# Gadersd/whisper-burn

Measured on AMD Instinct MI355X. Metric: real-time factor (audio-sec/wall-sec), higher is better.
Workload: dtype f32; 1 GPU; tiny.en, 30 s of 16 kHz audio per GPU per step, reference windowing (3 windows <= 14.9 s, 3 s overlap), HIP mel + encoder + KV-cached decode, greedy (beam_size 1), max_depth 100; windows=3, beam_size=1, max_depth=100, encoder_gemm_after_the_run=f16x3, parallelism=windows sharded over 1 GPU(s), 1 token all-gather

## Files before the change

### include/whisper_hip.h

```cpp
#ifndef WHISPER_HIP_H
#define WHISPER_HIP_H

#include <stdint.h>

#ifdef __cplusplus
extern "C" {
#endif

typedef enum wb_status {
  WB_OK = 0,
  WB_ERR_ARG = -1,
  WB_ERR_SHAPE = -2,
  WB_ERR_IO = -3,
  WB_ERR_HIP = -4,
  WB_ERR_OOM = -5,
  WB_ERR_STATE = -6
} wb_status;

enum { WB_F32 = 0,
       WB_BF16 = 1 };

typedef struct wb_model wb_model;
typedef struct wb_session wb_session;

// ... 119 lines not shown
                          void* user, int32_t* out_tokens, int32_t row_stride, int32_t* out_lens);

int wb_waveform_to_tokens(wb_model* m, const float* pcm, int64_t n, int sample_rate,
                          const wb_decode_params* p, const uint8_t* is_special, int win_begin,
                          int win_end, int32_t* win_tokens, int32_t row_stride, int32_t* win_lens,
                          int32_t* stitched, int64_t stitched_cap, int64_t* n_stitched);

int wb_waveform_to_tokens_dev(wb_model* m, const float* pcm_dev, int64_t n, int sample_rate,
                              const wb_decode_params* p, const uint8_t* is_special, int win_begin,
                              int win_end, int32_t* win_tokens, int32_t row_stride, int32_t* win_lens,
                              int32_t* stitched, int64_t stitched_cap, int64_t* n_stitched);

typedef int (*wb_allgather_fn)(void* user, const void* send, void* recv, int64_t bytes_per_rank);
typedef struct wb_comm wb_comm;
int wb_comm_unique_id(uint8_t* id128);
int wb_comm_init(const uint8_t* id128, int rank, int world, int device, wb_comm** out);
void wb_comm_free(wb_comm* c);
int wb_comm_allgather(void* comm, const void* send, void* recv, int64_t bytes_per_rank);

int wb_shard_partition(int64_t n_windows, int rank, int world, int64_t* lo, int64_t* hi);

int wb_waveform_to_tokens_sharded(wb_model* m, const float* pcm, int pcm_on_device, int64_t n, int sample_rate,
                                  const wb_decode_params* p, const uint8_t* is_special, int rank, int world,
                                  wb_allgather_fn allgather, void* user, int32_t* win_tokens, int32_t row_stride,
                                  int32_t* win_lens, int64_t win_cap, int32_t* stitched, int64_t stitched_cap,
                                  int64_t* n_stitched);

int64_t wb_window_extents(int64_t n_samples, int sample_rate, int64_t window_len, int overlap_seconds,
                          int64_t* starts, int64_t* lens, int64_t cap);

int wb_find_chunk_overlap(const int32_t* prev, int64_t n_prev, const int32_t* curr, int64_t n_curr,
                          int max_n_offsets, int min_n_overlaps, int64_t* prev_index,
                          int64_t* curr_index);

int wb_stitch_windows(const int32_t* win_tokens, int32_t row_stride, const int32_t* win_lens,
                      int n_windows, int max_n_offsets, int min_n_overlaps, int32_t* out,
                      int64_t cap, int64_t* n_out);

int wb_align_tokens(wb_model* m, const int32_t* tokens, int n, int L, const int32_t* lens, const float* enc, int C,
                    const int32_t* heads, int32_t n_heads, int32_t n_prefix, int32_t drop_last, int32_t filter_width,
                    int32_t* start_pos, float* matrix);
int wb_session_align(wb_session* s, const int32_t* tokens, int32_t row_stride, const int32_t* lens, const int32_t* heads,
                     int32_t n_heads, int32_t n_prefix, int32_t drop_last, int32_t filter_width, int32_t* start_pos,
                     float* matrix);
int wb_dtw_start_positions(int device, const float* x, int32_t N, int32_t C, int32_t* start_pos);
int wb_waveform_to_token_times(wb_model* m, const float* pcm, int64_t n, int sample_rate, const wb_decode_params* p,
                               const uint8_t* is_special, int win_begin, int win_end, int32_t* win_tokens,
                               int32_t row_stride, int32_t* win_lens, int32_t* stitched, int64_t stitched_cap,
                               int64_t* n_stitched, const int32_t* heads, int32_t n_heads, int32_t filter_width,
                               float* win_times, float* stitched_times);
int wb_stitch_windows_times(const int32_t* win_tokens, int32_t row_stride, const int32_t* win_lens, int n_windows,
                            int max_n_offsets, int min_n_overlaps, int32_t* out, int64_t cap, int64_t* n_out,
                            const float* win_times, float* out_times);

int wb_score_tokens(wb_model* m, const int32_t* tokens, int n, int L, const int32_t* lens, const float* enc, int C,
                    const uint8_t* is_special, int32_t mask_until_len, const int32_t* probe_ids, int32_t n_probe,
                    int32_t probe_pos, float* token_logprobs, float* probe_logprobs);
int wb_session_score(wb_session* s, const int32_t* tokens, int32_t row_stride, const int32_t* lens,
                     int32_t mask_until_len, const int32_t* probe_ids, int32_t n_probe, int32_t probe_pos,
                     float* token_logprobs, float* probe_logprobs);
int wb_waveform_detect_language(wb_model* m, const float* pcm, int64_t n, int sample_rate, int32_t padding,
                                int32_t tok_start_of_transcript, const int32_t* lang_ids, int32_t n_lang,
                                int32_t max_windows, float* win_probs, float* mean_probs, int32_t* best);
int wb_waveform_to_token_scores(wb_model* m, const float* pcm, int64_t n, int sample_rate, const wb_decode_params* p,
                                const uint8_t* is_special, int win_begin, int win_end, int32_t* win_tokens,
                                int32_t row_stride, int32_t* win_lens, int32_t* stitched, int64_t stitched_cap,
                                int64_t* n_stitched, int32_t tok_no_speech, float* win_logprobs,
                                float* stitched_logprobs, float* win_avg_logprob, float* win_no_speech_prob);
int wb_logprob_gather(int device, const float* h, int32_t R, int32_t d, const float* E, int32_t V, const float* mask,
                      const uint8_t* row_masked, const int32_t* target, const int32_t* probe_row,
                      const int32_t* probe_id, int32_t n_probe, int32_t v_splits, float* logprob, float* lse,
                      float* probe_lp);

typedef struct wb_sample_params {
  float temperature;
  int32_t best_of;
  uint64_t seed;
  int32_t attempt;
} wb_sample_params;
void wb_sample_params_default(wb_sample_params* p);
int wb_session_rewind(wb_session* s);
int wb_session_graph_count(const wb_session* s);
int64_t wb_session_graph_captures(const wb_session* s);
int wb_session_decode_sample(wb_session* s, const wb_decode_params* p, const wb_sample_params* sp, const int32_t* prompt,
                             int32_t prompt_len, const uint8_t* active, const int32_t* stream_ids, int32_t* out_tokens,
                             int32_t row_stride, int32_t* out_lens, double* out_sum_logprob, int32_t* out_best);

int wb_session_last_samples(wb_session* s, int32_t* tokens, int32_t row_stride, int32_t* lens);

enum { WB_FALLBACK_MAX_TEMPERATURES = 8 };
enum { WB_FALLBACK_ACCEPT = 0, WB_FALLBACK_RETRY = 1, WB_FALLBACK_NO_SPEECH = 2 };
typedef struct wb_fallback_params {
  float temperatures[WB_FALLBACK_MAX_TEMPERATURES];
  int32_t n_temperatures;
  int32_t best_of;
  float logprob_threshold;
  float no_speech_threshold;
  float compression_ratio_threshold;
  uint64_t seed;
  int32_t tok_no_speech;
} wb_fallback_params;
void wb_fallback_params_default(wb_fallback_params* p);
int wb_fallback_decide(const wb_fallback_params* fp, float avg_logprob, float no_speech_prob, float ratio);
typedef double (*wb_ratio_fn)(void* user, const int32_t* tokens, int32_t n);
int wb_waveform_to_tokens_fallback(wb_model* m, const float* pcm, int64_t n, int sample_rate, const wb_decode_params* p,
                                   const uint8_t* is_special, int win_begin, int win_end, int32_t* win_tokens,
                                   int32_t row_stride, int32_t* win_lens, int32_t* stitched, int64_t stitched_cap,
                                   int64_t* n_stitched, const wb_fallback_params* fp, wb_ratio_fn ratio, void* user,
                                   float* win_temperature, int32_t* win_status, float* win_avg_logprob,
                                   float* win_no_speech_prob, float* win_ratio, int32_t* win_attempts);
int wb_sample_rows(int device, const float* logits, int32_t R, int32_t ld, int32_t V, const float* mask,
                   const uint8_t* row_masked, const float* row_stats, float temperature, uint64_t seed, int32_t attempt,
                   const int32_t* stream, const int32_t* position, int32_t eot, int32_t* out_token, float* out_logprob,
                   int32_t* out_err);

int64_t wb_first_repetition_end(const int32_t* tokens, int64_t n, int64_t period);
int64_t wb_repetition_period(const int32_t* tokens, int64_t n, int64_t min_repetitions);
int wb_find_repeated_tokens_index(const int32_t* tokens, int64_t n, int64_t window_size, int64_t min_repeat_count,
                                  int64_t* first_repeat_index, int64_t* end);

int wb_mel_constants(double sample_rate, float* hann400, float* filters_80x201);

int wb_mel_dft_table(float* table_402x400);


int wb_profile_enable(int on);
int wb_profile_read(double* out8, int reset);

typedef struct wb_kernel_stat {
  char name[96];
  int64_t calls;
  double total_ms;
  double algo_bytes;
} wb_kernel_stat;
int wb_profile_kernels(wb_kernel_stat* out, int cap, int reset);

const char* wb_last_error(void);
const char* wb_version(void);

#ifdef __cplusplus
}
#endif
#endif
```

### rust/whisper-hip/src/ffi.rs

```rust
#![allow(non_camel_case_types)]
use std::os::raw::{c_char, c_double, c_float, c_int, c_void};

#[repr(C)]
pub struct wb_model {
    _private: [u8; 0],
}
#[repr(C)]
pub struct wb_session {
    _private: [u8; 0],
}
#[repr(C)]
pub struct wb_comm {
    _private: [u8; 0],
}

#[repr(C)]
#[derive(Default, Clone, Copy, Debug, PartialEq, Eq)]
pub struct wb_dims {
    pub n_mels: i32,
    pub n_audio_ctx: i32,
    pub n_audio_state: i32,
    pub n_audio_head: i32,
    pub n_audio_layer: i32,
    pub n_vocab: i32,
// ... 43 lines not shown
    pub tok_no_speech: i32,
}

pub type wb_ratio_fn = Option<unsafe extern "C" fn(user: *mut c_void, tokens: *const i32, n: i32) -> c_double>;

pub const WB_OK: c_int = 0;
pub const WB_ERR_ARG: c_int = -1;
pub const WB_ERR_SHAPE: c_int = -2;
pub const WB_ERR_IO: c_int = -3;
pub const WB_ERR_HIP: c_int = -4;
pub const WB_ERR_OOM: c_int = -5;
pub const WB_ERR_STATE: c_int = -6;
pub const WB_F32: c_int = 0;
pub const WB_BF16: c_int = 1;
pub const WB_FRONTEND_FFT: c_int = 0;
pub const WB_FRONTEND_REFERENCE: c_int = 1;

extern "C" {
    pub fn wb_model_load_dump_dir(dir: *const c_char, device: c_int, compute_dtype: c_int, out: *mut *mut wb_model) -> c_int;
    pub fn wb_model_load_burn_record(mpk_gz_path: *const c_char, cfg_path: *const c_char, device: c_int,
                                     compute_dtype: c_int, out: *mut *mut wb_model) -> c_int;
    pub fn wb_model_dims(m: *const wb_model, out: *mut wb_dims) -> c_int;
    pub fn wb_model_free(m: *mut wb_model);
    pub fn wb_model_set_frame_limit(m: *mut wb_model, whisper_geometry: c_int) -> c_int;
    pub fn wb_model_set_frontend(m: *mut wb_model, frontend: c_int) -> c_int;
    pub fn wb_model_frontend(m: *const wb_model) -> c_int;
    pub fn wb_model_encoder_gemm(m: *const wb_model) -> c_int;
    pub fn wb_model_decoder_gemm(m: *const wb_model) -> c_int;
    pub fn wb_max_waveform_samples(n_frame_max: i64) -> i64;
    pub fn wb_prep_audio(device: c_int, pcm: *const c_float, n: i64, sample_rate: c_double, mel: *mut c_float,
                         n_frames: *mut i64) -> c_int;
    pub fn wb_prep_audio_frontend(device: c_int, pcm: *const c_float, n: i64, sample_rate: c_double, mel: *mut c_float,
                                  n_frames: *mut i64, frontend: c_int) -> c_int;
    pub fn wb_mel_dft_table(table_402x400: *mut c_float) -> c_int;
    pub fn wb_forward_encoder(m: *mut wb_model, mel: *const c_float, b: c_int, t: c_int, out: *mut c_float) -> c_int;
    pub fn wb_forward_decoder(m: *mut wb_model, tokens: *const i32, n: c_int, l: c_int, enc: *const c_float, c: c_int,
                              logits: *mut c_float) -> c_int;
    pub fn wb_forward(m: *mut wb_model, mel: *const c_float, b: c_int, t: c_int, tokens: *const i32, l: c_int,
                      logits: *mut c_float) -> c_int;
    pub fn wb_decode_params_default(p: *mut wb_decode_params);
    pub fn wb_window_extents(n_samples: i64, sample_rate: c_int, window_len: i64, overlap_seconds: c_int,
                             starts: *mut i64, lens: *mut i64, cap: i64) -> i64;
    pub fn wb_waveform_to_tokens(m: *mut wb_model, pcm: *const c_float, n: i64, sample_rate: c_int,
                                 p: *const wb_decode_params, is_special: *const u8, win_begin: c_int, win_end: c_int,
                                 win_tokens: *mut i32, row_stride: i32, win_lens: *mut i32, stitched: *mut i32,
                                 stitched_cap: i64, n_stitched: *mut i64) -> c_int;
    pub fn wb_align_tokens(m: *mut wb_model, tokens: *const i32, n: c_int, L: c_int, lens: *const i32, enc: *const c_float,
                           C: c_int, heads: *const i32, n_heads: i32, n_prefix: i32, drop_last: i32, filter_width: i32,
                           start_pos: *mut i32, matrix: *mut c_float) -> c_int;
    pub fn wb_session_align(s: *mut wb_session, tokens: *const i32, row_stride: i32, lens: *const i32, heads: *const i32,
                            n_heads: i32, n_prefix: i32, drop_last: i32, filter_width: i32, start_pos: *mut i32,
                            matrix: *mut c_float) -> c_int;
    pub fn wb_dtw_start_positions(device: c_int, x: *const c_float, N: i32, C: i32, start_pos: *mut i32) -> c_int;
    pub fn wb_waveform_to_token_times(m: *mut wb_model, pcm: *const c_float, n: i64, sample_rate: c_int,
                                      p: *const wb_decode_params, is_special: *const u8, win_begin: c_int, win_end: c_int,
                                      win_tokens: *mut i32, row_stride: i32, win_lens: *mut i32, stitched: *mut i32,
                                      stitched_cap: i64, n_stitched: *mut i64, heads: *const i32, n_heads: i32,
                                      filter_width: i32, win_times: *mut c_float, stitched_times: *mut c_float) -> c_int;
    pub fn wb_stitch_windows_times(win_tokens: *const i32, row_stride: i32, win_lens: *const i32, n_windows: c_int,
                                   max_n_offsets: c_int, min_n_overlaps: c_int, out: *mut i32, cap: i64, n_out: *mut i64,
                                   win_times: *const c_float, out_times: *mut c_float) -> c_int;
    pub fn wb_score_tokens(m: *mut wb_model, tokens: *const i32, n: c_int, L: c_int, lens: *const i32, enc: *const c_float,
                           C: c_int, is_special: *const u8, mask_until_len: i32, probe_ids: *const i32, n_probe: i32,
                           probe_pos: i32, token_logprobs: *mut c_float, probe_logprobs: *mut c_float) -> c_int;
    pub fn wb_session_score(s: *mut wb_session, tokens: *const i32, row_stride: i32, lens: *const i32, mask_until_len: i32,
                            probe_ids: *const i32, n_probe: i32, probe_pos: i32, token_logprobs: *mut c_float,
                            probe_logprobs: *mut c_float) -> c_int;
    pub fn wb_waveform_detect_language(m: *mut wb_model, pcm: *const c_float, n: i64, sample_rate: c_int, padding: i32,
                                       tok_start_of_transcript: i32, lang_ids: *const i32, n_lang: i32, max_windows: i32,
                                       win_probs: *mut c_float, mean_probs: *mut c_float, best: *mut i32) -> c_int;
    pub fn wb_waveform_to_token_scores(m: *mut wb_model, pcm: *const c_float, n: i64, sample_rate: c_int,
                                       p: *const wb_decode_params, is_special: *const u8, win_begin: c_int, win_end: c_int,
                                       win_tokens: *mut i32, row_stride: i32, win_lens: *mut i32, stitched: *mut i32,
                                       stitched_cap: i64, n_stitched: *mut i64, tok_no_speech: i32,
                                       win_logprobs: *mut c_float, stitched_logprobs: *mut c_float,
                                       win_avg_logprob: *mut c_float, win_no_speech_prob: *mut c_float) -> c_int;
    pub fn wb_logprob_gather(device: c_int, h: *const c_float, R: i32, d: i32, E: *const c_float, V: i32,
                             mask: *const c_float, row_masked: *const u8, target: *const i32, probe_row: *const i32,
                             probe_id: *const i32, n_probe: i32, v_splits: i32, logprob: *mut c_float, lse: *mut c_float,
                             probe_lp: *mut c_float) -> c_int;
    pub fn wb_session_rewind(s: *mut wb_session) -> c_int;
    pub fn wb_session_graph_count(s: *const wb_session) -> c_int;
    pub fn wb_session_graph_captures(s: *const wb_session) -> i64;
    pub fn wb_session_last_samples(s: *mut wb_session, tokens: *mut i32, row_stride: i32, lens: *mut i32) -> c_int;
    pub fn wb_sample_rows(device: c_int, logits: *const c_float, R: i32, ld: i32, V: i32, mask: *const c_float,
                          row_masked: *const u8, row_stats: *const c_float, temperature: c_float, seed: u64, attempt: i32,
                          stream: *const i32, position: *const i32, eot: i32, out_token: *mut i32,
                          out_logprob: *mut c_float, out_err: *mut i32) -> c_int;
    pub fn wb_session_begin(m: *mut wb_model, pcm: *const c_float, n_pcm: i64, starts: *const i64, lens: *const i64,
                            n_windows: c_int, max_beams: c_int, padding: c_int, out: *mut *mut wb_session) -> c_int;
    pub fn wb_session_set_special_mask(s: *mut wb_session, is_special: *const u8) -> c_int;
    pub fn wb_session_step(s: *mut wb_session, new_tokens: *const i32, parent: *const i32, window: *const i32, n: c_int,
                           apply_special_mask: c_int, k: c_int, top_ids: *mut i32, top_logprobs: *mut c_float) -> c_int;
    pub fn wb_session_decode(s: *mut wb_session, p: *const wb_decode_params, out_tokens: *mut i32, row_stride: i32,
                             out_lens: *mut i32) -> c_int;
    pub fn wb_session_free(s: *mut wb_session);
    pub fn wb_wav_read_f32(path: *const c_char, out: *mut c_float, capacity: i64, n_samples: *mut i64) -> c_int;
    pub fn wb_wav_read_f32_any_rate(path: *const c_char, out: *mut c_float, capacity: i64, n_samples: *mut i64) -> c_int;
    pub fn wb_resample_len(n_in: i64, rate_in: i32, rate_out: i32) -> i64;
    pub fn wb_resample_dev(device: c_int, src_dev: *const c_float, n_in: i64, rate_in: i32, rate_out: i32,
                           dst_dev: *mut c_float, capacity: i64, n_out: *mut i64) -> c_int;
    pub fn wb_comm_unique_id(id128: *mut u8) -> c_int;
    pub fn wb_comm_init(id128: *const u8, rank: c_int, world: c_int, device: c_int, out: *mut *mut wb_comm) -> c_int;
    pub fn wb_comm_free(c: *mut wb_comm);
    pub fn wb_comm_allgather(comm: *mut c_void, send: *const c_void, recv: *mut c_void, bytes_per_rank: i64) -> c_int;
    pub fn wb_shard_partition(n_windows: i64, rank: c_int, world: c_int, lo: *mut i64, hi: *mut i64) -> c_int;
    pub fn wb_waveform_to_tokens_sharded(m: *mut wb_model, pcm: *const c_float, pcm_on_device: c_int, n: i64,
                                         sample_rate: c_int, p: *const wb_decode_params, is_special: *const u8,
                                         rank: c_int, world: c_int, allgather: wb_allgather_fn, user: *mut c_void,
                                         win_tokens: *mut i32, row_stride: i32, win_lens: *mut i32, win_cap: i64,
                                         stitched: *mut i32, stitched_cap: i64, n_stitched: *mut i64) -> c_int;
    pub fn wb_last_error() -> *const c_char;
    pub fn wb_version() -> *const c_char;
}

extern "C" {
    pub fn wb_sample_params_default(p: *mut wb_sample_params);
    pub fn wb_session_decode_sample(s: *mut wb_session, p: *const wb_decode_params, sp: *const wb_sample_params,
                                    prompt: *const i32, prompt_len: i32, active: *const u8, stream_ids: *const i32,
                                    out_tokens: *mut i32, row_stride: i32, out_lens: *mut i32,
                                    out_sum_logprob: *mut c_double, out_best: *mut i32) -> c_int;
    pub fn wb_fallback_params_default(p: *mut wb_fallback_params);
    pub fn wb_fallback_decide(fp: *const wb_fallback_params, avg_logprob: c_float, no_speech_prob: c_float,
                              ratio: c_float) -> c_int;
    pub fn wb_waveform_to_tokens_fallback(m: *mut wb_model, pcm: *const c_float, n: i64, sample_rate: c_int,
                                          p: *const wb_decode_params, is_special: *const u8, win_begin: c_int,
                                          win_end: c_int, win_tokens: *mut i32, row_stride: i32, win_lens: *mut i32,
                                          stitched: *mut i32, stitched_cap: i64, n_stitched: *mut i64,
                                          fp: *const wb_fallback_params, ratio: wb_ratio_fn, user: *mut c_void,
                                          win_temperature: *mut c_float, win_status: *mut i32,
                                          win_avg_logprob: *mut c_float, win_no_speech_prob: *mut c_float,
                                          win_ratio: *mut c_float, win_attempts: *mut i32) -> c_int;
}

pub type wb_allgather_fn = Option<unsafe extern "C" fn(user: *mut c_void, send: *const c_void, recv: *mut c_void,
                                                       bytes_per_rank: i64) -> c_int>;

pub unsafe extern "C" fn wb_comm_allgather_thunk(user: *mut c_void, send: *const c_void, recv: *mut c_void,
                                                  bytes_per_rank: i64) -> c_int {
    wb_comm_allgather(user, send, recv, bytes_per_rank)
}

pub type wb_user = *mut c_void;
```

### whisper-burn_amd/csrc/decode.h

```cpp
#pragma once
#include <hip/hip_runtime.h>
#include <hip/hip_ext.h>
#include <stdint.h>

#include <algorithm>

#include "kernels.h"
#include "wb_internal.h"

namespace wb {

constexpr int MAX_BEAMS = 8;
constexpr int TOPK_MAX = 8;
constexpr int CA_STRIDE = 66;
constexpr int CA_NCH_MAX = 12;
constexpr int TS_STRIDE = 2 + 2 * TOPK_MAX;
constexpr int GV_CT = 128;
constexpr int GV_CT_LOGITS = 128;
constexpr int KS_MAX = 16;

enum { ST_N = 0, ST_STEP = 1, ST_HDR = 4 };
enum { GC_STEP = 0, GC_NDONE = 1, GC_ALLDONE = 2, GC_BAD = 3, GC_HDR = 4 };
struct StepLayout {
  int S = 0, W = 0;
// ... 153 lines not shown
};
void launch_sample_rows(hipStream_t st, const SampleRowsArgs& a);

struct MlpFusedArgs {
  const int* st = nullptr; int S = 0, d = 0;
  const float* x_in = nullptr; const float* pend = nullptr; int KSp = 0; const float* pbias = nullptr; float* x_out = nullptr;
  int n_head = 0, n_chunks = 0;
  const float* ln_g = nullptr; const float* ln_b = nullptr; float ln_eps = 0.f; int ln_inside = 0;
  const float* W1 = nullptr; int ld1 = 0; const float* b1 = nullptr;
  const float* W2 = nullptr;
  float* P = nullptr;
  unsigned long long* stamps = nullptr;
  int row0 = 0;
  const void* g_x_in = nullptr; const void* g_pend = nullptr; void* g_x_out = nullptr; void* g_P = nullptr;
};
struct AttnFusedArgs {
  const int* st = nullptr; StepLayout lay; int S = 0, d = 0, n_head = 0;
  const float* x_in = nullptr; const float* pend = nullptr; int KSp = 0; const float* pbias = nullptr; float* x_out = nullptr;
  const float* ln_g = nullptr; const float* ln_b = nullptr; float ln_eps = 0.f; int ln_inside = 0;
  const float* Wqkv = nullptr; int ldqkv = 0; const float* bqkv = nullptr; float scale = 0.f;
  float* Kc = nullptr; float* Vc = nullptr; const int* tabs = nullptr; int Lmax = 0;
  const float* Wo = nullptr;
  float* P = nullptr;
  unsigned long long* stamps = nullptr;
  const void* g_x_in = nullptr; const void* g_pend = nullptr; void* g_x_out = nullptr; void* g_P = nullptr;
};
struct CrossFusedArgs {
  const int* st = nullptr; StepLayout lay; int S = 0, d = 0, n_head = 0;
  const float* x_in = nullptr; const float* pend = nullptr; int KSp = 0; const float* pbias = nullptr; float* x_out = nullptr;
  const float* ln_g = nullptr; const float* ln_b = nullptr; float ln_eps = 0.f; int ln_inside = 0;
  const float* Wq = nullptr; const float* bq = nullptr; float scale = 0.f;
  const float* ckv = nullptr; int ldkv = 0, koff = 0;
  const int* win_row0 = nullptr; const int* win_C = nullptr;
  int n_pass = 1;
  const float* Wo = nullptr;
  float* P = nullptr;
  unsigned long long* stamps = nullptr;
  const void* g_x_in = nullptr; const void* g_pend = nullptr; void* g_x_out = nullptr; void* g_P = nullptr;
};
struct SkinnyArgs {
  const float* A = nullptr; int lda = 0;
  const float* B = nullptr; int ldb = 0;
  int M = 0, N = 0, K = 0, ksplit = 1;
  float* P = nullptr; int plane = 0;
  const uint16_t* Bh = nullptr; const uint16_t* Bl = nullptr;
  int* range_flag = nullptr;
  const int* st = nullptr;
};
void launch_split_weight_f16_tiles(hipStream_t st, const float* W, int K, int N, uint16_t* hi, uint16_t* lo);
int skinny_ksplit(int K, int N, int max_ks, int max_rows);
bool skinny_supported(int M, int K, int N);
int launch_dec_skinny_gemm(hipStream_t st, const SkinnyArgs& a);

struct PsLayerArgs { AttnFusedArgs attn; CrossFusedArgs cross; MlpFusedArgs mlp; };
enum { PSR_ATTN = 0, PSR_CROSS = 1, PSR_MLP = 2, PSR_LOGITS = 3, PSR_MERGE = 4, PSR_FINLN = 5 };
struct PsRole { int kind, layer, a, b; };
constexpr int PS_MAX_FORCED = 8;
struct PersistArgs {
  const PsLayerArgs* layers = nullptr;
  const PsRole* roles = nullptr; int n_roles = 0;
  const int* role_off = nullptr;
  const int* res_role = nullptr;
  int n_logits_roles = 0;
  int n_layer = 0, n_rows = 0, S = 0, d = 0, n_head = 0, nb_mlp = 0;
  int n_pass = 1;
  int* ctl = nullptr;
  int step0 = 0, n_steps = 0;
  int n_forced = 0; int forced[PS_MAX_FORCED] = {0, 0, 0, 0, 0, 0, 0, 0};
  int mask_until_len = 0;
  const void* x_fin = nullptr; const void* P2 = nullptr; const float* b2_last = nullptr;
  void* g_xn = nullptr;
  unsigned tag_base = 0;
  const float* ln_g = nullptr; const float* ln_b = nullptr; float ln_eps = 0.f; int ln_inside = 0;
  const float* Et = nullptr; int vocab_ld = 0, V = 0; const float* mask = nullptr;
  float* tstats = nullptr; int n_tiles = 0;
  int* gctl = nullptr; int* gtok = nullptr; int Lmax = 0, eot = 0;
  const float* E = nullptr; const float* pos = nullptr; void* x0 = nullptr; int* tabs = nullptr;
  int* dead = nullptr;
  unsigned long long* stamps = nullptr;
};
int ps_ctl_ints(int S, int n_layer);
bool dec_persist_supported(int d, int n_rows, int max_keys);
int dec_persist_resident_slots(int d, int n_rows, int max_keys);
int dec_persist_max_grid(int device, int d, int n_rows, int max_keys);
int launch_dec_persist(hipStream_t st, const PersistArgs& a, int grid);
void launch_ps_seed(hipStream_t st, const float* x, int n, void* gx, unsigned tag);

#if defined(HIPEMU) && !defined(HIPEMU_PROD_GEOMETRY)
constexpr int CROSS_FUSED_MAX_C = 384;
#else
constexpr int CROSS_FUSED_MAX_C = 768;
#endif
constexpr int CROSS_FUSED_MAX_PASSES = 2;
void launch_dec_cross_fused(hipStream_t st, const CrossFusedArgs& a, int n_rows_hint);
bool dec_fused_supported(int d);
int dec_mlp_fused_planes(int d);
void launch_dec_mlp_fused(hipStream_t st, const MlpFusedArgs& a, int n_rows_hint);
void launch_dec_attn_fused(hipStream_t st, const AttnFusedArgs& a, int n_rows_hint);

}
```

### whisper-burn_amd/csrc/decode_chain.cpp

```cpp
#include <climits>
#include <cstring>

#include "decode_step.h"
#include "handoff.h"
#include "switches.h"

using namespace wb;

namespace wb {

static int run_persistent_chain(wb_session* s, int eot, int max_depth, int mask_until_len, const int32_t* forced, int n_forced,
                                int* steps_done, bool* fell_back) {
  *fell_back = false;
  WB_REQUIRE(n_forced >= 0 && n_forced <= PS_MAX_FORCED, WB_ERR_ARG, "persistent decode: %d prompt steps", n_forced);
  const char* inject = sw::persist_inject_fail();
  wb_model* m = s->m;
  const wb_dims& D = m->dims;
  const int d = D.n_text_state, H = D.n_text_head, NL = D.n_text_layer, V = D.n_vocab, S = s->S, W = s->W;
  const StepLayout& L = s->lay;
  hipStream_t st = s->st;
  const int NB = dec_mlp_fused_planes(d);
  const int n_tiles = (V + 127) / 128;
  const size_t pool = (size_t)s->Lmax * S;
  const int ldkv = 2 * d;
  WB_REQUIRE(NB <= 32 && H <= 8, WB_ERR_SHAPE, "persistent decode: more planes than its folds hold");
  WB_TRY(s->ps_gx.ensure_zeroed(((size_t)2 * S + 8) * d * 8, st));
  WB_TRY(s->ps_gpa.ensure_zeroed(((size_t)H * S + 8) * d * 8, st));
  WB_TRY(s->ps_gpc.ensure_zeroed(((size_t)H * S + 8) * d * 8, st));
  WB_TRY(s->ps_gp2.ensure_zeroed(((size_t)NB * S + 8) * d * 8, st));
  WB_TRY(s->ps_gxn.ensure_zeroed(((size_t)S + 8) * d * 8, st));
  if (((s->ps_launches + 1) & 0xffffu) == 0) {
    for (DevMem* b : {&s->ps_gx, &s->ps_gpa, &s->ps_gpc, &s->ps_gp2, &s->ps_gxn}) WB_HIP(hipMemsetAsync(b->p, 0, b->bytes, st));
    s->ps_launches++;
  }
  const unsigned tag_base = ((++s->ps_launches) & 0xffffu) << 16;
  char* gxb[2] = {static_cast<char*>(s->ps_gx.p), static_cast<char*>(s->ps_gx.p) + (size_t)S * d * 8};
  std::vector<PsLayerArgs> la(NL);
  float* xb[2] = {s->x.as<float>(), s->x.as<float>() + (size_t)S * d};
  int xi = 0;
  for (int l = 0; l < NL; l++) {
    const DecBlockW& b = m->dec[l];
    AttnFusedArgs& fa = la[l].attn;
    fa.st = s->state.as<int>(); fa.lay = L; fa.S = S; fa.d = d; fa.n_head = H;
    fa.x_in = xb[xi]; fa.pend = l == 0 ? nullptr : s->P2.as<float>(); fa.KSp = l == 0 ? 0 : NB;
    fa.pbias = l == 0 ? nullptr : m->dec[l - 1].mlp2.b; fa.x_out = xb[xi ^ 1];
    fa.ln_g = b.ln1.g; fa.ln_b = b.ln1.b; fa.ln_eps = b.ln1.eps; fa.ln_inside = m->ln_eps_inside_sqrt;
    fa.Wqkv = b.qkv.w; fa.ldqkv = b.qkv.n; fa.bqkv = b.qkv.b; fa.scale = m->qk_scale;
    fa.Kc = s->kc.as<float>() + (size_t)l * pool * d; fa.Vc = s->vc.as<float>() + (size_t)l * pool * d;
    fa.tabs = s->tabs.as<int>(); fa.Lmax = s->Lmax; fa.Wo = b.out.w; fa.P = s->Pa.as<float>();
    fa.g_x_in = gxb[xi]; fa.g_pend = l == 0 ? nullptr : s->ps_gp2.p; fa.g_x_out = gxb[xi ^ 1]; fa.g_P = s->ps_gpa.p;
    xi ^= 1;
    CrossFusedArgs& ca = la[l].cross;
    ca.st = s->state.as<int>(); ca.lay = L; ca.S = S; ca.d = d; ca.n_head = H;
    ca.x_in = xb[xi]; ca.pend = s->Pa.as<float>(); ca.KSp = H; ca.pbias = b.out.b; ca.x_out = xb[xi ^ 1];
    ca.ln_g = b.ln2.g; ca.ln_b = b.ln2.b; ca.ln_eps = b.ln2.eps; ca.ln_inside = m->ln_eps_inside_sqrt;
    ca.Wq = b.cq.w; ca.bq = b.cq.b; ca.scale = m->qk_scale;
    ca.ckv = s->ckv.as<float>() + (size_t)l * s->enc_rows * 2 * d; ca.ldkv = ldkv; ca.koff = 0;
    ca.win_row0 = s->win_meta.as<int>(); ca.win_C = s->win_meta.as<int>() + W;
    ca.Wo = b.cout.w; ca.P = s->Pc.as<float>();
    ca.n_pass = s->maxC > CROSS_FUSED_MAX_C ? 2 : 1;
    ca.g_x_in = gxb[xi]; ca.g_pend = s->ps_gpa.p; ca.g_x_out = gxb[xi ^ 1]; ca.g_P = s->ps_gpc.p;
    xi ^= 1;
    MlpFusedArgs& ma = la[l].mlp;
    ma.st = s->state.as<int>(); ma.S = S; ma.d = d;
    ma.x_in = xb[xi]; ma.pend = s->Pc.as<float>(); ma.KSp = H; ma.pbias = b.cout.b; ma.x_out = xb[xi ^ 1];
    ma.ln_g = b.ln3.g; ma.ln_b = b.ln3.b; ma.ln_eps = b.ln3.eps; ma.ln_inside = m->ln_eps_inside_sqrt;
    ma.W1 = b.mlp1.w; ma.ld1 = b.mlp1.n; ma.b1 = b.mlp1.b; ma.W2 = b.mlp2.w; ma.P = s->P2.as<float>();
    ma.g_x_in = gxb[xi]; ma.g_pend = s->ps_gpc.p; ma.g_x_out = gxb[xi ^ 1]; ma.g_P = s->ps_gp2.p;
    xi ^= 1;
  }
  std::vector<PsRole> lr;
  for (int l = 0; l < NL; l++) {
    for (int r = 0; r < W; r++) for (int h = 0; h < H; h++) lr.push_back(PsRole{PSR_ATTN, l, h, r});
    for (int r = 0; r < W; r++) for (int h = 0; h < H; h++) lr.push_back(PsRole{PSR_CROSS, l, h, r});
    for (int j = 0; j < NB; j++) lr.push_back(PsRole{PSR_MLP, l, j, 0});
  }
  const int grid = std::max(1, std::min(s->ps_grid, (int)lr.size() + n_tiles + 2 * W));
  std::vector<std::vector<PsRole>> deal(grid);
  for (size_t i = 0; i < lr.size(); i++) deal[i % grid].push_back(lr[i]);
  std::vector<int> cand;
  for (int b = 0; b < grid; b++) {
    bool early = false;
    for (const PsRole& r : deal[b]) early |= r.layer == 0 && (r.kind == PSR_ATTN || r.kind == PSR_CROSS);
    if (!early) cand.push_back(b);
  }
  if ((int)cand.size() * 4 < n_tiles) { cand.clear(); for (int b = 0; b < grid; b++) cand.push_back(b); }
  std::vector<char> is_fin(grid, 0);
  {
    std::vector<int> order(grid);
    for (int b = 0; b < grid; b++) order[b] = b;
    std::stable_sort(order.begin(), order.end(), [&](int x, int y) { return deal[x].size() < deal[y].size(); });
    for (int r = 0; r < W; r++) { deal[order[r % grid]].push_back(PsRole{PSR_FINLN, 0, 0, r}); is_fin[order[r % grid]] = 1; }
  }
  if ((int)cand.size() > 2 * W) cand.erase(std::remove_if(cand.begin(), cand.end(), [&](int b) { return is_fin[b] != 0; }), cand.end());
  std::stable_sort(cand.begin(), cand.end(), [&](int x, int y) { return deal[x].size() < deal[y].size(); });
  const int tpb = (n_tiles + (int)cand.size() - 1) / (int)cand.size();
  const int n_lg = (n_tiles + tpb - 1) / tpb;
  for (int q = 0; q < n_lg; q++)
    deal[cand[q]].push_back(PsRole{PSR_LOGITS, q, q * tpb, std::min(tpb, n_tiles - q * tpb)});
  {
    std::vector<int> order(grid);
    for (int b = 0; b < grid; b++) order[b] = b;
    std::stable_sort(order.begin(), order.end(), [&](int x, int y) { return deal[x].size() < deal[y].size(); });
    for (int r = 0; r < W; r++) deal[order[r % grid]].push_back(PsRole{PSR_MERGE, 0, 0, r});
  }
  std::vector<PsRole> roles;
  std::vector<int> role_off(grid + 1, 0);
  for (int b = 0; b < grid; b++) {
    role_off[b] = (int)roles.size();
    roles.insert(roles.end(), deal[b].begin(), deal[b].end());
  }
  role_off[grid] = (int)roles.size();
  const char* res_sw = sw::persist_resident();
  const bool res_on = !(res_sw && res_sw[0] == '0') && dec_persist_resident_slots(d, W, s->maxC) > 0;
  std::vector<int> res_role(grid, -1);
  int n_res = 0;
  if (res_on)
    for (int b = 0; b < grid; b++) {
      int n_layer_roles = 0, at = -1;
      for (int i = role_off[b]; i < role_off[b + 1]; i++)
        if (roles[i].kind <= PSR_MLP) { n_layer_roles++; at = i; }
      if (n_layer_roles == 1 && roles[at].kind != PSR_MLP) { res_role[b] = at; n_res++; }
    }
  if (res_sw && !strcmp(res_sw, "log")) fprintf(stderr, "persist resident blocks: %d of %d\n", n_res, grid);
  const int n_ctl = ps_ctl_ints(S, NL);
  WB_TRY(s->ps_layers.ensure(la.size() * sizeof(PsLayerArgs)));
  WB_TRY(s->ps_roles.ensure(roles.size() * sizeof(PsRole) + (role_off.size() + res_role.size()) * 4));
  WB_TRY(s->ps_ctl.ensure((size_t)n_ctl * 4));
  WB_TRY(s->ps_dead.ensure((size_t)S * 4));
  WB_TRY(s->ps_tstats.ensure((size_t)S * n_tiles * 2 * 4));
  std::vector<int> ctl0(n_ctl, 0);
  ctl0[HX_STOP] = INT_MAX;
  WB_HIP(hipMemcpyAsync(s->ps_layers.p, la.data(), la.size() * sizeof(PsLayerArgs), hipMemcpyHostToDevice, st));
  WB_HIP(hipMemcpyAsync(s->ps_roles.p, roles.data(), roles.size() * sizeof(PsRole), hipMemcpyHostToDevice, st));
  WB_HIP(hipMemcpyAsync(static_cast<char*>(s->ps_roles.p) + roles.size() * sizeof(PsRole) + role_off.size() * 4, res_role.data(),
                        res_role.size() * 4, hipMemcpyHostToDevice, st));
  WB_HIP(hipMemcpyAsync(static_cast<char*>(s->ps_roles.p) + roles.size() * sizeof(PsRole), role_off.data(), role_off.size() * 4,
                        hipMemcpyHostToDevice, st));
  WB_HIP(hipMemcpyAsync(s->ps_ctl.p, ctl0.data(), (size_t)n_ctl * 4, hipMemcpyHostToDevice, st));
  WB_HIP(hipMemsetAsync(s->ps_dead.p, 0, (size_t)S * 4, st));
  PersistArgs a;
  a.layers = s->ps_layers.as<PsLayerArgs>(); a.roles = s->ps_roles.as<PsRole>(); a.n_roles = (int)roles.size();
  a.role_off = reinterpret_cast<const int*>(static_cast<char*>(s->ps_roles.p) + roles.size() * sizeof(PsRole));
  if (n_res > 0) a.res_role = a.role_off + role_off.size();
  a.n_logits_roles = n_lg;
  a.n_layer = NL; a.n_rows = W; a.S = S; a.d = d; a.n_head = H; a.nb_mlp = NB;
  a.n_pass = s->maxC > CROSS_FUSED_MAX_C ? 2 : 1;
  a.ctl = s->ps_ctl.as<int>(); a.step0 = s->step; a.n_steps = n_forced + max_depth; a.mask_until_len = mask_until_len;
  a.n_forced = n_forced;
  for (int i = 0; i < n_forced; i++) a.forced[i] = forced[i];
  a.g_xn = s->ps_gxn.p;
  a.x_fin = gxb[xi]; a.P2 = s->ps_gp2.p; a.b2_last = m->dec[NL - 1].mlp2.b; a.tag_base = tag_base;
  a.ln_g = m->ln_dec.g; a.ln_b = m->ln_dec.b; a.ln_eps = m->ln_dec.eps; a.ln_inside = m->ln_eps_inside_sqrt;
  a.Et = m->tok_emb_t; a.vocab_ld = m->vocab_ld; a.V = V; a.mask = s->mask.as<float>();
  a.tstats = s->ps_tstats.as<float>(); a.n_tiles = n_tiles;
  a.gctl = s->gctl.as<int>(); a.gtok = s->gtok.as<int>(); a.Lmax = s->Lmax; a.eot = eot;
  a.E = m->tok_emb; a.pos = m->dec_pos; a.x0 = gxb[0]; a.tabs = s->tabs.as<int>(); a.dead = s->ps_dead.as<int>();
  const char* stamps_path = sw::ps_stamps();
  const size_t n_stamps = stamps_path ? (size_t)(n_forced + max_depth) * roles.size() * 8 : 0;
  if (n_stamps) {
    WB_TRY(s->ps_stamps.ensure(n_stamps * 8));
    WB_HIP(hipMemsetAsync(s->ps_stamps.p, 0, n_stamps * 8, st));
    a.stamps = s->ps_stamps.as<unsigned long long>();
  }
  WB_REQUIRE(3 * NL * (n_forced + max_depth + 1) + 4 < 0x10000, WB_ERR_SHAPE,
             "persistent decode: %d layers x %d steps do not fit the 16-bit granule tags", NL, max_depth);
  launch_dec_prepare(st, reinterpret_cast<const int*>(s->host_block_dev), s->state.as<int>(), L, W, s->tabs.as<int>(),
                     s->Lmax, m->tok_emb, m->dec_pos, d, s->x.as<float>(), s->gctl.as<int>());
  launch_ps_seed(st, s->x.as<float>(), W * d, gxb[0], tag_base + 1u);
  WB_HIP(hipStreamSynchronize(st));
  hipEvent_t e0 = nullptr, e1 = nullptr;
  prof_tag(KC_PERSIST, 0.0);
  const bool timed = prof_take_events(&e0, &e1);
  if (timed) WB_HIP(hipEventRecord(e0, st));
  const bool refused = (inject && !strcmp(inject, "launch")) || launch_dec_persist(st, a, grid) != 0;
  if (timed) WB_HIP(hipEventRecord(e1, st));
  if (refused) {
    (void)hipGetLastError();
    s->ps_grid = 0;
    *fell_back = true;
    *steps_done = 0;
    return WB_OK;
  }
  std::vector<int> ctl(n_ctl);
  WB_HIP(hipMemcpyAsync(ctl.data(), s->ps_ctl.p, (size_t)n_ctl * 4, hipMemcpyDeviceToHost, st));
  int gstep = 0;
  WB_HIP(hipMemcpyAsync(&gstep, s->gctl.as<int>() + GC_STEP, 4, hipMemcpyDeviceToHost, st));
  WB_HIP(hipStreamSynchronize(st));
  if (ctl[HX_ERR] != 0 && gstep == s->step) {
    s->ps_grid = 0;
    *fell_back = true;
    *steps_done = 0;
    return WB_OK;
  }
  WB_REQUIRE(ctl[HX_ERR] == 0, WB_ERR_HIP, "persistent decode: a wait gave up (counter %d) at step %d", ctl[HX_ERR] - 1, gstep);
  if (n_stamps) {
    std::vector<unsigned long long> hs(n_stamps);
    WB_HIP(hipMemcpy(hs.data(), s->ps_stamps.p, n_stamps * 8, hipMemcpyDeviceToHost));
    if (FILE* f = fopen(stamps_path, "wb")) {
      const int hdr[4] = {n_forced + max_depth, (int)roles.size(), grid, 8};
      fwrite(hdr, 4, 4, f);
      std::vector<int> kinds(roles.size());
      for (size_t i = 0; i < roles.size(); i++)
        kinds[i] = roles[i].kind | ((roles[i].kind <= PSR_MLP ? roles[i].layer : 0) << 8) |
                   ((roles[i].kind == PSR_LOGITS ? 0 : roles[i].b) << 16);
      fwrite(kinds.data(), 4, kinds.size(), f);
      fwrite(hs.data(), 8, hs.size(), f);
      fclose(f);
    }
  }
  *steps_done = std::max(0, std::min(n_forced + max_depth, gstep - s->step));
  return WB_OK;
}

int session_greedy_chain(wb_session* s, const int32_t* prompt, int eot, int max_depth, int mask_until_len, int prompt_len,
                         int32_t* out_tokens, int32_t row_stride, int32_t* out_lens) {
  wb_model* m = s->m;
  const int S = s->S, W = s->W;
  WB_REQUIRE(S == W, WB_ERR_STATE, "chained greedy decode needs max_beams == 1");
  WB_REQUIRE(prompt && prompt_len >= 1, WB_ERR_ARG, "chained greedy decode: empty prompt");
  WB_REQUIRE(s->step == 0 || (s->prev_n == W && s->step == prompt_len - 1), WB_ERR_STATE,
             "chained greedy decode: the session is neither fresh nor prefilled");
  const int n_forced_max = prompt_len - 1;
  auto host_prefill = [&]() -> int {
    std::vector<int32_t> tok(W), par(W), win(W);
    for (int t = s->step; t < prompt_len - 1; t++) {
      for (int w = 0; w < W; w++) { tok[w] = prompt[t]; par[w] = t == 0 ? -1 : w; win[w] = w; }
      WB_TRY(wb_session_step(s, tok.data(), par.data(), win.data(), W, 0, 0, nullptr, nullptr));
    }
    return WB_OK;
  };
  WB_REQUIRE(s->has_mask || mask_until_len < prompt_len || max_depth == 0, WB_ERR_STATE,
             "wb_session_decode: special mask not set");
  const int asked_depth = max_depth;
  max_depth = std::min(max_depth, s->Lmax - (prompt_len - 1));
  WB_HIP(hipSetDevice(m->device));
  hipStream_t st = s->st;
  const size_t ctl_ints = GC_HDR + 3 * (size_t)S;
  WB_TRY(s->gctl.ensure(ctl_ints * 4));
  WB_TRY(s->gtok.ensure(((size_t)S * s->Lmax + 1) * 4));
  std::vector<int> ctl(ctl_ints, 0);
  auto seed_ctl = [&]() -> int {
    std::fill(ctl.begin(), ctl.end(), 0);
    ctl[GC_STEP] = s->step;
    for (int i = 0; i < W; i++) ctl[GC_HDR + i] = prompt[s->step];
    WB_HIP(hipMemcpyAsync(s->gctl.p, ctl.data(), ctl_ints * 4, hipMemcpyHostToDevice, st));
    WB_HIP(hipStreamSynchronize(st));
    return WB_OK;
  };
  const StepPlan plan = plan_step(s, W, false);
  const int n_launch = plan.n_launch;
  const bool fuse_ln = plan.fuse_ln;
  const int chunk = 16;
  int depth = 0;
  bool persist = plan.persist && max_depth > 0;
  if (persist) {
    if (s->ps_grid < 0) s->ps_grid = dec_persist_max_grid(m->device, m->dims.n_text_state, W, s->maxC);
    persist = s->ps_grid > 0;
  }
  int n_forced = 0;
  if (persist && sw::persist_prefill() && s->step == 0 && n_forced_max <= PS_MAX_FORCED && s->has_mask) n_forced = n_forced_max;
  if (n_forced == 0) WB_TRY(host_prefill());
  WB_TRY(seed_ctl());
  ScopedTimer tm(st, 3);
  if (persist) {
    bool fell_back = false;
    WB_TRY(run_persistent_chain(s, eot, max_depth, mask_until_len, prompt + s->step + 1, n_forced, &depth, &fell_back));
    if (fell_back) {
      persist = false;
      depth = 0;
      WB_TRY(host_prefill());
      WB_TRY(seed_ctl());
      n_forced = 0;
    } else {
      if (profile().on) profile().ms[4] += depth;
      depth -= n_forced;
      s->step += n_forced;
      s->prev_n = W;
      s->prev_win.resize(W);
      for (int w = 0; w < W; w++) s->prev_win[w] = w;
    }
  }
  if (!persist) {
  if (fuse_ln)
    launch_dec_prepare(st, reinterpret_cast<const int*>(s->host_block_dev), s->state.as<int>(), s->lay, n_launch,
                       s->tabs.as<int>(), s->Lmax, m->tok_emb, m->dec_pos, m->dims.n_text_state, s->x.as<float>(),
                       s->gctl.as<int>());
  const bool speculate = fuse_ln && sw::speculate();
  if (speculate && !s->st2) {
    WB_HIP(hipStreamCreateWithFlags(&s->st2, hipStreamNonBlocking));
    WB_HIP(hipEventCreateWithFlags(&s->ev_seg, hipEventDisableTiming));
  }
  auto enqueue_segment = [&](int* enq) -> int {
    int n = 0;
    while (depth + n < max_depth && n < chunk) {
      const int d0 = depth + n;
      const int use_mask = (prompt_len + d0) <= mask_until_len ? 1 : 0;
      const int run = (!use_mask && max_depth - d0 >= chunk) ? chunk : 1;
      StepCall call;
      call.k = 1; call.use_mask = use_mask; call.chained = true; call.eot = eot; call.reps = run;
      WB_TRY(launch_step(s, plan, call));
      if (profile().on) profile().ms[4] += run;
      n += run;
    }
    *enq = n;
    return WB_OK;
  };
  auto read_flags = [&](bool behind_event) -> int {
    if (behind_event) {
      WB_HIP(hipStreamWaitEvent(s->st2, s->ev_seg, 0));
      WB_HIP(hipMemcpyAsync(ctl.data(), s->gctl.p, ctl_ints * 4, hipMemcpyDeviceToHost, s->st2));
      WB_HIP(hipStreamSynchronize(s->st2));
    } else {
      WB_HIP(hipMemcpyAsync(ctl.data(), s->gctl.p, ctl_ints * 4, hipMemcpyDeviceToHost, st));
      WB_HIP(hipStreamSynchronize(st));
    }
    return WB_OK;
  };
  auto all_done = [&]() {
    bool d = true;
    for (int i = 0; i < W; i++) d = d && ctl[GC_HDR + S + i] != 0;
    return d;
  };
  const bool poll = fuse_ln && sw::poll() && !profile().on;
  volatile int* hfl = reinterpret_cast<volatile int*>(s->host_block + s->chain_flags_off);
  if (poll) for (int i = 0; i < 2 * S; i++) hfl[i] = 0;
  auto wait_flags = [&](int want_step, bool* done) -> int {
    for (long spins = 0;; spins++) {
      bool ready = true;
      for (int i = 0; i < W && ready; i++) ready = hfl[2 * i] >= want_step;
      if (ready) break;
      bool fin = true;
      for (int i = 0; i < W && fin; i++) fin = hfl[2 * i + 1] != 0;
      if (fin) break;
      if ((spins & 0xfff) == 0xfff) {
        const hipError_t q = hipStreamQuery(st);
        if (q == hipSuccess) {
          bool r2 = true;
          for (int i = 0; i < W && r2; i++) r2 = hfl[2 * i] >= want_step;
          if (r2) break;
          bool all = true;
          for (int i = 0; i < W; i++) all = all && hfl[2 * i + 1] != 0;
          if (all) break;
          set_error("chained decode: the device stopped at step %d of %d", (int)hfl[0], want_step);
          return WB_ERR_HIP;
        }
        if (q != hipErrorNotReady) { set_error("chained decode: %s", hipGetErrorString(q)); return WB_ERR_HIP; }
      }
    }
    __atomic_thread_fence(__ATOMIC_ACQUIRE);
    bool all = true;
    for (int i = 0; i < W; i++) all = all && hfl[2 * i + 1] != 0;
    *done = all;
    return WB_OK;
  };
  if (!speculate) {
    while (depth < max_depth) {
      int n = 0;
      WB_TRY(enqueue_segment(&n));
      depth += n;
      if (poll) {
        bool done = false;
        WB_TRY(wait_flags(s->step + depth, &done));
        if (done) break;
      } else {
        WB_TRY(read_flags(false));
        if (all_done()) break;
      }
    }
  } else {
    int n_cur = 0;
    WB_TRY(enqueue_segment(&n_cur));
    depth += n_cur;
    while (true) {
      WB_HIP(hipEventRecord(s->ev_seg, st));
      int n_next = 0;
      if (depth < max_depth) { WB_TRY(enqueue_segment(&n_next)); depth += n_next; }
      WB_TRY(read_flags(true));
      if (all_done() || n_next == 0) break;
    }
    WB_HIP(hipStreamSynchronize(st));
  }
  }
  tm.stop();
  std::vector<int> toks((size_t)S * s->Lmax + 1);
  WB_HIP(hipMemcpyAsync(ctl.data(), s->gctl.p, ctl_ints * 4, hipMemcpyDeviceToHost, st));
  WB_HIP(hipMemcpyAsync(toks.data(), s->gtok.p, toks.size() * 4, hipMemcpyDeviceToHost, st));
  WB_HIP(hipStreamSynchronize(st));
  tm.collect();
  WB_TRY(dec_split_check(s));
  WB_REQUIRE(ctl[GC_BAD] == 0, WB_ERR_STATE, "a decode step produced a row without a finite log-prob (NaN logits: non-finite "
             "weights or activations); its window was ended on <|endoftext|> on the device and the rows of this call are invalid");
  for (int w = 0; w < W; w++) {
    int len = ctl[GC_HDR + 2 * S + w];
    if (len < prompt_len) len = prompt_len;
    len = std::min(len, prompt_len + max_depth);
    WB_REQUIRE(len <= row_stride, WB_ERR_ARG, "row_stride too small");
    for (int p = prompt_len; p < len; p++) out_tokens[(size_t)w * row_stride + p] = toks[(size_t)w * s->Lmax + p];
    out_lens[w] = len;
  }
  if (profile().on && !persist && s->prof_cls_cross >= 0 && s->prof_cls_self >= 0) {
    const int dm = m->dims.n_text_state, NL = m->dims.n_text_layer;
    double dead_ckv = 0, dead_self = 0;
    for (int w = 0; w < W; w++) {
      const int live = std::max(0, std::min(out_lens[w] - prompt_len, depth));
      for (int t = live; t < depth; t++) { dead_ckv += 8.0 * s->C[w] * dm; dead_self += 8.0 * (s->step + t + 1) * dm; }
    }
    prof_adjust_bytes(s->prof_cls_cross, -(double)NL * dead_ckv);
    prof_adjust_bytes(s->prof_cls_self, -(double)NL * dead_self);
  }
  if (profile().on && persist) {
    const double dm = m->dims.n_text_state, NL = m->dims.n_text_layer;
    double bytes = (double)(depth + n_forced) * 4.0 * NL * 14.0 * dm * dm + (double)depth * 4.0 * (double)m->dims.n_vocab * dm;
    for (int w = 0; w < W; w++)
      for (int t = 0; t < n_forced; t++) bytes += NL * (8.0 * s->C[w] * dm + 8.0 * (t + 1) * dm);
    for (int w = 0; w < W; w++) {
      const int live = std::max(0, std::min(out_lens[w] - prompt_len, depth));
      for (int t = 0; t < live; t++) bytes += NL * (8.0 * s->C[w] * dm + 8.0 * (s->step + t + 1) * dm);
    }
    prof_adjust_bytes(KC_PERSIST, bytes);
  }
  s->prof_step_off = 0;
  s->step += depth;
  s->prev_len.assign(W, s->step);
  s->last_had_logits = 0;
  if (max_depth < asked_depth)
    for (int w = 0; w < W; w++)
      WB_REQUIRE(ctl[GC_HDR + S + w] != 0, WB_ERR_SHAPE, "Token sequence length %d must not exceed %d.", s->Lmax + 1,
                 s->Lmax);
  return WB_OK;
}
}
```

### whisper-burn_amd/csrc/decode_fused_bodies.h

```cpp
#pragma once
#include <hip/hip_runtime.h>

#include "decode.h"
#include "handoff.h"
#include "wave_ops.h"

namespace wb {
namespace fused {

struct PsStep {
  const unsigned* ctr = nullptr; unsigned target = 0; int ctr_index = 0;
  const int* ctl = nullptr;
  int step = 0;
  int n_rows = 0;
  const int* dead = nullptr;
  int* lds_flag = nullptr;
  unsigned long long* stamp = nullptr;
  int n_ctr = 1;
  unsigned tag_in = 0, tag_out = 0;
  bool known_dead = false;
  mutable bool saw_dead = false;
};
constexpr int PS_STAMPS = 8;
__device__ __forceinline__ void ps_stamp(const PsStep& ps, int k) {
// ... 12 lines not shown
                               : hx_wait(ps.ctr, ps.target, ps.ctl, ps.step, ps.ctr_index, ps.lds_flag);
  ps_stamp(ps, 1);
  return ok;
}
__device__ __forceinline__ bool ps_sweep_retry(unsigned& sweeps, const PsStep& ps) {
  if ((sweeps & 31u) == 31u &&
      (__hip_atomic_load(ps.ctl + HX_STOP, __ATOMIC_RELAXED, __HIP_MEMORY_SCOPE_AGENT) <= ps.step ||
       __hip_atomic_load(ps.ctl + HX_ERR, __ATOMIC_RELAXED, __HIP_MEMORY_SCOPE_AGENT) != 0)) return true;
  if (++sweeps > HX_SWEEP_LIMIT) {
    __hip_atomic_store(const_cast<int*>(ps.ctl) + HX_ERR, 5000 + ps.ctr_index, __ATOMIC_RELAXED, __HIP_MEMORY_SCOPE_AGENT);
    return true;
  }
  __builtin_amdgcn_s_sleep(1);
  return false;
}
__device__ __forceinline__ bool ps_sweeps_ok(const PsStep& ps) { return *ps.lds_flag != 0; }
template <int UNITS>
__device__ __forceinline__ void ps_nap() {
#if !defined(WB_PS_DRY) || defined(WB_PS_DRY_NAPS)
#ifndef WB_PS_NAP_ADJ
#define WB_PS_NAP_ADJ 0
#endif
#pragma unroll
  for (int i = 0; i < UNITS + (WB_PS_NAP_ADJ); i++) __builtin_amdgcn_s_sleep(64);
#endif
}

#ifdef WB_STAMPS
#define WB_STAMP_DECL unsigned long long stamp_buf[16];
#define WB_STAMP(i) do { if (threadIdx.x == 0 && blockIdx.x == 0 && blockIdx.y == 0) sm.stamp_buf[i] = wall_clock64(); } while (0)
#define WB_STAMP_FLUSH(a, n) do { if (threadIdx.x == 0 && blockIdx.x == 0 && blockIdx.y == 0 && (a).stamps) for (int _i = 0; _i < (n); _i++) (a).stamps[_i] = sm.stamp_buf[_i]; } while (0)
#else
#define WB_STAMP_DECL
#define WB_STAMP(i) do {} while (0)
#define WB_STAMP_FLUSH(a, n) do {} while (0)
#endif

constexpr int FD_MAX = 512;
constexpr int FA_MAXPOS = 448;


constexpr int ROLE_NT = 512;
template <int MR, int DPL, bool REC>
struct MlpLds {
  static constexpr int d = 64 * DPL, HS = 64, G = d / 4 <= 32 ? 8 : 4;
  alignas(16) float hs[MR][d];
  alignas(16) float red[8][MR][HS];
  alignas(16) float hid[MR][HS];
  alignas(16) float obuf[(G - 1) * MR * d];
  float mlb[REC ? MR : 1][48][2];
  float coef[REC ? MR : 1][48];
  WB_STAMP_DECL
};
template <int DPL>
struct AttnLds {
  static constexpr int d = 64 * DPL, G = d / 4 <= 32 ? 8 : 4;
  static constexpr int RED = (8 * 192 > (G - 1) * d) ? 8 * 192 : (G - 1) * d;
  alignas(16) float hs[d];
  alignas(16) float red[RED];
  alignas(16) float qkv[192];
  int tbs[FA_MAXPOS];
  float sc[FA_MAXPOS];
  alignas(16) float part[32][64];
  alignas(16) float att[64];
  WB_STAMP_DECL
};
template <int DPL, int NP>
struct CrossLds {
  static constexpr int d = 64 * DPL, G = d / 4 <= 32 ? 8 : 4, CMAX = NP * CROSS_FUSED_MAX_C;
  alignas(16) float hs[d];
  alignas(16) float red[8][64];
  alignas(16) float qv[64];
  float sc[CMAX];
  float pbuf[CMAX];
  alignas(16) float part[32][64];
  alignas(16) float att[64];
  alignas(16) float obuf[(G - 1) * d];
};

template <int DPL, int NP, int RS>
struct ResGeom {
  static constexpr int d = 64 * DPL, G = d / 4 <= 32 ? 8 : 4, RPG = 64 / G;
  static constexpr int KW = d / 8, RK = DPL >= 6 ? 8 : 16, NIT = KW / RK;
  static constexpr int NRND = (NIT - 2 < RS / RK ? NIT - 2 : RS / RK) > 0 ? (NIT - 2 < RS / RK ? NIT - 2 : RS / RK) : 0;
  static constexpr int WO_A = NRND * RK;
  static constexpr int NWO_A = RS - WO_A < RPG ? RS - WO_A : RPG;
  static constexpr int SL = 4, NTILE = CROSS_FUSED_MAX_C / 128;
  static constexpr int NVT = NP > 1 ? 0 : (RS / SL < NTILE ? RS / SL : NTILE);
  static constexpr int WO_X = NVT * SL;
  static constexpr int NWO_X = NP > 1 ? 0 : (RS - WO_X < RPG ? RS - WO_X : RPG);
  static_assert(RS >= 0 && WO_A + NWO_A <= RS && WO_X + NWO_X <= RS, "resident slots");
};
__device__ __forceinline__ float4 res_ld(const float4* res, int slot, int tid) { return res[slot * ROLE_NT + tid]; }
__device__ __forceinline__ void res_st(float4* res, int slot, int tid, const float4& v) { res[slot * ROLE_NT + tid] = v; }

__device__ __forceinline__ float gelu_erf_f(float x) {
  return 0.5f * x * (1.0f + erff(x * 0.70710678118654752440f));
}

template <int DPL>
__device__ __forceinline__ void fold_ln_row(const float* __restrict__ x_in, const float* __restrict__ pend, int KSp,
                                            int64_t plane, const float* __restrict__ pbias, float* __restrict__ x_out,
                                            const float* __restrict__ g, const float* __restrict__ b, float eps,
                                            int eps_inside, int d, int row, int lane, float* __restrict__ out) {
  int co[DPL];
#pragma unroll
  for (int i = 0; i < DPL; i++) co[i] = lane + (64 * i < d ? 64 * i : 0);
  float gv[DPL], bv[DPL], v[DPL];
  const float* xr = x_in + (int64_t)row * d;
#pragma unroll
  for (int i = 0; i < DPL; i++) { gv[i] = g[co[i]]; bv[i] = b[co[i]]; v[i] = xr[co[i]]; }
  if (KSp > 0) {
    float acc[DPL];
#pragma unroll
    for (int i = 0; i < DPL; i++) acc[i] = pbias[co[i]];
    const float* pp = pend + (int64_t)row * d;
    constexpr int CH = DPL <= 6 ? 8 : 4;
    for (int sp = 0; sp < KSp; sp += CH) {
      float t[CH][DPL];
#pragma unroll
      for (int j = 0; j < CH; j++) {
        const float* pj = pp + (int64_t)min(sp + j, KSp - 1) * plane;
#pragma unroll
        for (int i = 0; i < DPL; i++) t[j][i] = pj[co[i]];
      }
#pragma unroll
      for (int j = 0; j < CH; j++) {
        const bool live = sp + j < KSp;
#pragma unroll
        for (int i = 0; i < DPL; i++) acc[i] += live ? t[j][i] : 0.f;
      }
    }
#pragma unroll
    for (int i = 0; i < DPL; i++) v[i] = v[i] + acc[i];
  }
  float s = 0.f;
#pragma unroll
  for (int i = 0; i < DPL; i++) {
    if (64 * i < d) { s += v[i]; if (x_out) x_out[(int64_t)row * d + co[i]] = v[i]; }
  }
  const float mean = wave_sum(s) / (float)d;
  float q = 0.f;
#pragma unroll
  for (int i = 0; i < DPL; i++) {
    if (64 * i < d) { const float t = v[i] - mean; q += t * t; }
  }
  const float var = wave_sum(q) / (float)d;
  const float denom = eps_inside ? sqrtf(var + eps) : (sqrtf(var) + eps);
#pragma unroll
  for (int i = 0; i < DPL; i++) {
    const int c = lane + 64 * i;
    if (c < d) out[c] = (v[i] - mean) / denom * gv[i] + bv[i];
  }
}

template <int NT, int MR, int EPT, int PCH>
__device__ __forceinline__ void fold_rows(const float* __restrict__ x_in, const float* __restrict__ pend, int KSp,
                                          int64_t plane, const float* __restrict__ pbias, int d, int tid,
                                          float (&v)[EPT]) {
  int off[EPT], col[EPT];
#pragma unroll
  for (int i = 0; i < EPT; i++) {
    int e = tid + NT * i;
    if (e >= MR * d) e = tid;
    off[i] = e; col[i] = e % d;
  }
#pragma unroll
  for (int i = 0; i < EPT; i++) v[i] = x_in[off[i]];
  if (KSp > 0) {
    float acc[EPT];
#pragma unroll
    for (int i = 0; i < EPT; i++) acc[i] = pbias[col[i]];
    for (int sp = 0; sp < KSp; sp += PCH) {
      float t[PCH][EPT];
#pragma unroll
      for (int j = 0; j < PCH; j++) {
        const float* pj = pend + (int64_t)min(sp + j, KSp - 1) * plane;
// ... 480 lines not shown
        if (ok) {
          v = gx.v;
          if (a.KSp > 0) {
#pragma unroll
            for (int j = 0; j < FP; j++) accp += (j < a.KSp) ? g[j].v : 0.f;
            v += accp;
          }
          break;
        }
        if (ps_sweep_retry(sweeps, ps)) { *ps.lds_flag = 0; break; }
      }
      xfold = v;
      if (tid < d) hs[tid] = v;
    } else {
    float v = a.x_in[(int64_t)r * d + c];
    constexpr int FP = 32;
    float t[FP];
    float accp = 0.f;
    if (a.KSp > 0) {
      accp = gld(a.pbias + c);
#pragma unroll
      for (int j = 0; j < FP; j++) t[j] = pp[(int64_t)min(j, a.KSp - 1) * plane];
    }
    load_weights();
    if (r >= n_rows || dead) return true;
    if (a.KSp > 0) {
#pragma unroll
      for (int j = 0; j < FP; j++) accp += (j < a.KSp) ? t[j] : 0.f;
      for (int sp = FP; sp < a.KSp; sp += FP) {
#pragma unroll
        for (int j = 0; j < FP; j++) t[j] = pp[(int64_t)min(sp + j, a.KSp - 1) * plane];
#pragma unroll
        for (int j = 0; j < FP; j++) accp += (sp + j < a.KSp) ? t[j] : 0.f;
      }
      v += accp;
    }
    xfold = v;
    if (tid < d) hs[tid] = v;
    }
  }
  if constexpr (!PS) qbias = tid < 192 ? a.bqkv[(tid >> 6) * d + h * 64 + (tid & 63)] : 0.f;
  if constexpr (!PS) load_cache_tile();
  WB_STAMP(1);
  if constexpr (PS) ps_stamp(ps, 2);
  __syncthreads();
  if constexpr (PS) { if (!ps_sweeps_ok(ps)) return false; }
#if defined(WB_PS_DRY)
  if constexpr (PS) {
    if (tid < d / 4) { const Buf16 pgo(a.g_P); st_gran4(pgo, (uint32_t)((h * a.S + r) * d + tid * 4), ps.tag_out, make_float4(0.f, 0.f, 0.f, 0.f)); }
    if (h == 0 && tid < d) { const Buf16 xgo(a.g_x_out); st_gran(xgo, (uint32_t)(r * d + tid), ps.tag_out, xfold); }
    return true;
  }
#endif
  float xn_own;
  {
    float mean, denom;
    ln_stats_lds<DPL>(hs, d, lane, a.ln_eps, a.ln_inside, mean, denom);
    xn_own = (hs[own_col] - mean) / denom * g_own + b_own;
  }
  if constexpr (PS) ps_stamp_fine(ps, 4);
  WB_STAMP(2);
  const int nres = (RG::NRND > 0 && res != nullptr) ? RG::NRND : 0;
  const int nreg = NIT - nres;
  float acc[4] = {0.f, 0.f, 0.f, 0.f};
#pragma unroll 1
  for (int n = 0; n < nreg; n += 2) {
#pragma unroll
    for (int b = 0; b < 2; b++) {
      if (n + b < nreg) {
        const int kb = RK * (n + b < 2 ? n + b : n + b + nres);
#pragma unroll
        for (int j = 0; j < RK; j++) {
          const float xv = __int_as_float(__builtin_amdgcn_readlane(__float_as_int(xn_own), kb + j));
          acc[0] += xv * wr[b][j].x; acc[1] += xv * wr[b][j].y; acc[2] += xv * wr[b][j].z; acc[3] += xv * wr[b][j].w;
        }
        if (n + b + 2 < nreg) load_round(wr[b], n + b + 2 + nres);
      }
      if constexpr (RG::NRND > 0) {
        if (b == 1 && n == 0 && nres > 0) {
#pragma unroll 1
          for (int q = 0; q < RG::NRND; q++) {
            float4 wl[RK];
#pragma unroll
            for (int j = 0; j < RK; j++) wl[j] = res_ld(res, q * RK + j, tid);
            const int kb = RK * (2 + q);
#pragma unroll
            for (int j = 0; j < RK; j++) {
              const float xv = __int_as_float(__builtin_amdgcn_readlane(__float_as_int(xn_own), kb + j));
              acc[0] += xv * wl[j].x; acc[1] += xv * wl[j].y; acc[2] += xv * wl[j].z; acc[3] += xv * wl[j].w;
            }
          }
        }
      }
    }
  }
  WB_STAMP(3);
  if constexpr (PS) ps_stamp(ps, 3);
  __syncthreads();
  const int cf = tid % CF, jg = tid / CF;
  const bool p5 = jg < G;
  const int jb = (p5 ? jg : 0) * RPG;
  float4 wo[RPG];
  {
    const float* wp = a.Wo + (int64_t)(h * 64 + jb) * d + cf * 4;
    if (RG::NWO_A == 0 || res == nullptr) {
#pragma unroll
      for (int i = 0; i < RG::NWO_A; i++) wo[i] = ld_w4(wp + (int64_t)i * d);
    }
#pragma unroll
    for (int i = RG::NWO_A; i < RPG; i++) wo[i] = ld_w4(wp + (int64_t)i * d);
  }
  if (seg_ok) *reinterpret_cast<float4*>(&red[wave * 192 + seg * 64 + c4]) = make_float4(acc[0], acc[1], acc[2], acc[3]);
  __syncthreads();
  if (tid < 192) {
    float v = 0.f;
#pragma unroll
    for (int w8 = 0; w8 < 8; w8++) v += red[w8 * 192 + tid];
    v += qbias;
    if (tid < 128) v *= a.scale;
    qkv[tid] = v;
  }
  __syncthreads();
  if constexpr (PS) ps_stamp_fine(ps, 5);
  WB_STAMP(4);
  {
    const float4 q4 = *reinterpret_cast<const float4*>(&qkv[pq4]);
    auto row_dot = [&](const float4& k4) {
      float s = q4.x * k4.x + q4.y * k4.y + q4.z * k4.z + q4.w * k4.w;
      s += dpp_f<DPP_QUAD_XOR1, 0xF>(0.f, s);
      s += dpp_f<DPP_QUAD_XOR2, 0xF>(0.f, s);
      s += dpp_f<DPP_ROW_HALF_MIRROR, 0xF>(0.f, s);
      s += dpp_f<DPP_ROW_MIRROR, 0xF>(0.f, s);
      return s;
    };
#pragma unroll
    for (int i = 0; i < PSL; i++) {
      const int p = rg + 32 * i;
      const float s = row_dot(kc[i]);
      if ((tid & 15) == 0 && p < npast) sc[p] = s;
    }
    for (int t0 = PT; t0 < npast; t0 += PT) {
      float4 kt[PSL];
#pragma unroll
      for (int i = 0; i < PSL; i++) {
        const int p = min(t0 + rg + 32 * i, npast - 1);
        int sl;
        if constexpr (PS) sl = p * a.lay.S + r; else sl = tbs[p];
        kt[i] = ld_f4<PS>(a.Kc, kbuf, (uint32_t)(sl * d + h * 64 + pq4));
      }
#pragma unroll
      for (int i = 0; i < PSL; i++) {
        const int p = t0 + rg + 32 * i;
        const float s = row_dot(kt[i]);
        if ((tid & 15) == 0 && p < npast) sc[p] = s;
      }
    }
    if (wave == 7) {
      const float s = wave_sum(qkv[lane] * qkv[64 + lane]);
      if (lane == 0) sc[npast] = s;
    }
  }
  __syncthreads();
  WB_STAMP(5);
  if constexpr (PS) ps_stamp(ps, 4);
  float m = -INFINITY;
  for (int p = lane; p < len; p += 64) m = fmaxf(m, sc[p]);
  m = wave_max(m);
  float l = 0.f;
  for (int p = lane; p < len; p += 64) l += expf(sc[p] - m);
  l = wave_sum(l);
  {
    float4 o = make_float4(0.f, 0.f, 0.f, 0.f);
#pragma unroll
    for (int i = 0; i < PSL; i++) {
      const int p = rg + 32 * i;
      const float pk = p < npast ? expf(sc[p] - m) : 0.f;
      o.x += pk * vc[i].x; o.y += pk * vc[i].y; o.z += pk * vc[i].z; o.w += pk * vc[i].w;
    }
    for (int t0 = PT; t0 < npast; t0 += PT) {
      float4 vt[PSL];
#pragma unroll
      for (int i = 0; i < PSL; i++) {
        const int p = min(t0 + rg + 32 * i, npast - 1);
        int sl;
        if constexpr (PS) sl = p * a.lay.S + r; else sl = tbs[p];
        vt[i] = ld_f4<PS>(a.Vc, vbuf, (uint32_t)(sl * d + h * 64 + pq4));
      }
#pragma unroll
      for (int i = 0; i < PSL; i++) {
        const int p = t0 + rg + 32 * i;
        const float pk = p < npast ? expf(sc[p] - m) : 0.f;
        o.x += pk * vt[i].x; o.y += pk * vt[i].y; o.z += pk * vt[i].z; o.w += pk * vt[i].w;
      }
    }
    *reinterpret_cast<float4*>(&part[rg][pq4]) = o;
  }
  __syncthreads();
  if (tid < 64) {
    float v = 0.f;
#pragma unroll
    for (int g2 = 0; g2 < 32; g2++) v += part[g2][tid];
    v += expf(sc[npast] - m) * qkv[128 + tid];
    att[tid] = v / l;
  }
  __syncthreads();
  WB_STAMP(6);
  if constexpr (PS) ps_stamp(ps, 5);
  if constexpr (RG::NWO_A > 0) {
    if (res != nullptr) {
#pragma unroll
      for (int i = 0; i < RG::NWO_A; i++) wo[i] = res_ld(res, RG::WO_A + i, tid);
    }
  }
  float ov[4] = {0.f, 0.f, 0.f, 0.f};
#pragma unroll
  for (int i = 0; i < RPG; i++) {
    const float av = att[jb + i];
    ov[0] += av * wo[i].x; ov[1] += av * wo[i].y; ov[2] += av * wo[i].z; ov[3] += av * wo[i].w;
  }
  if (p5 && jg > 0)
    *reinterpret_cast<float4*>(&red[(jg - 1) * d + cf * 4]) = make_float4(ov[0], ov[1], ov[2], ov[3]);
  __syncthreads();
  if (jg == 0) {
#pragma unroll
    for (int g2 = 1; g2 < G; g2++) {
      const float4 t = *reinterpret_cast<const float4*>(&red[(g2 - 1) * d + cf * 4]);
      ov[0] += t.x; ov[1] += t.y; ov[2] += t.z; ov[3] += t.w;
    }
    if constexpr (PS) {
      const Buf16 pgo(a.g_P);
      st_gran4(pgo, (uint32_t)((h * a.S + r) * d + cf * 4), ps.tag_out, make_float4(ov[0], ov[1], ov[2], ov[3]));
    } else {
      *reinterpret_cast<float4*>(&a.P[((int64_t)h * a.S + r) * d + cf * 4]) = make_float4(ov[0], ov[1], ov[2], ov[3]);
    }
  }
  if (tid >= 64 && tid < 192) {
    float* dst = (tid < 128 ? a.Kc : a.Vc) + (int64_t)slot_new * d + h * 64 + (tid & 63);
    st_f<PS>(dst, qkv[tid]);
  }
  if (h == 0 && tid < d) {
    if constexpr (PS) { const Buf16 xgo(a.g_x_out); st_gran(xgo, (uint32_t)(r * d + tid), ps.tag_out, xfold); }
    else a.x_out[(int64_t)r * d + tid] = xfold;
  }
  WB_STAMP(7);
  WB_STAMP_FLUSH(a, 8);
  return true;
}

template <int DPL, int RS>
__device__ __forceinline__ void dec_attn_res_fill(const AttnFusedArgs& a, const int h, float4* res) {
  using RG = ResGeom<DPL, 1, RS>;
  constexpr int d = 64 * DPL, KW = d / 8, RK = RG::RK, CF = d / 4, G = RG::G, RPG = RG::RPG;
  const int tid = role_tid<true>(), lane = tid & 63, wave = tid >> 6;
  const int seg = lane >> 4, c4 = (lane & 15) * 4;
  const float* wq = a.Wqkv + (int64_t)(wave * KW) * a.ldqkv + (seg < 3 ? seg : 0) * d + h * 64 + c4;
#pragma unroll 1
  for (int q = 0; q < RG::NRND; q++) {
    float4 w[RK];
#pragma unroll
    for (int j = 0; j < RK; j++) w[j] = ld_w4(wq + (int64_t)(RK * (2 + q) + j) * a.ldqkv);
#pragma unroll
    for (int j = 0; j < RK; j++) res_st(res, q * RK + j, tid, w[j]);
  }
  if constexpr (RG::NWO_A > 0) {
    const int cf = tid % CF, jg = tid / CF;
    const int jb = (jg < G ? jg : 0) * RPG;
    const float* wp = a.Wo + (int64_t)(h * 64 + jb) * d + cf * 4;
    float4 w[RG::NWO_A];
#pragma unroll
    for (int i = 0; i < RG::NWO_A; i++) w[i] = ld_w4(wp + (int64_t)i * d);
#pragma unroll
    for (int i = 0; i < RG::NWO_A; i++) res_st(res, RG::WO_A + i, tid, w[i]);
  }
}

template <int DPL, bool PS, int NP = 1, int RS = 0>
__device__ __forceinline__ bool dec_cross_body(const CrossFusedArgs& a, const int h, const int r, const PsStep& ps,
                                               CrossLds<DPL, NP>& sm, const float4* res = nullptr) {
  constexpr int NT = 512;
  constexpr int PASS_C = CROSS_FUSED_MAX_C, CMAX = NP * PASS_C;
  constexpr int d = 64 * DPL;
  constexpr int NWQ = d / 32;
  constexpr int CF = d / 4;
  constexpr int G = CF <= 32 ? 8 : 4;
  constexpr int RPG = 64 / G;
  constexpr int KT = 128, NTILE = CROSS_FUSED_MAX_C / KT, SL = KT * 16 / NT;
  static_assert(CROSS_FUSED_MAX_C % KT == 0 && SL * NT == KT * 16, "tile geometry");
  using RG = ResGeom<DPL, NP, PS ? RS : 0>;
  static_assert(G == CrossLds<DPL, NP>::G && CMAX == CrossLds<DPL, NP>::CMAX && RG::SL == SL && RG::NTILE == NTILE && RG::RPG == RPG &&
                NT == ROLE_NT, "LDS struct / resident geometry");
  auto& hs = sm.hs; auto& red = sm.red; auto& qv = sm.qv; auto& sc = sm.sc; auto& pbuf = sm.pbuf; auto& part = sm.part; auto& att = sm.att;
  auto& obuf = sm.obuf;
  const bool res_v = RG::NVT > 0 && res != nullptr;
  const int tid = role_tid<PS>(), lane = tid & 63, wave = tid >> 6;
  if (h >= a.n_head) return true;
  int n_live, w_row, dead;
  if constexpr (PS) { n_live = ps.n_rows; w_row = r; dead = 0; }
  else {
    n_live = a.st[ST_N]; w_row = a.st[a.lay.win + r];
    dead = a.st[a.lay.dead + r];
  }
  const int wi8 = min(lane & 7, a.lay.W - 1);
  const int vC8 = gld(a.win_C + wi8), vR8 = gld(a.win_row0 + wi8);
  float xfold;
  const int rg = tid >> 4, c4 = (tid & 15) * 4;
  constexpr int NOWN = 4 * NWQ;
  const int own_col = 4 * wave + (lane & 3) + 32 * ((lane < NOWN ? lane : 0) >> 2);
  float g_own = 0.f, b_own = 0.f;
  float4 wqr[NWQ];
  float4 kv[NTILE][SL];
  const float* Kh; const float* Vh; int C;
  float qbias = 0.f;
  auto load_weights = [&]() {
    g_own = gld(a.ln_g + own_col); b_own = gld(a.ln_b + own_col);
    if constexpr (PS) { if (tid < 64) qbias = gld(a.bq + h * 64 + tid); }
    {
      const float* wp = a.Wq + (int64_t)rg * d + h * 64 + c4;
#pragma unroll
      for (int i = 0; i < NWQ; i++) wqr[i] = ld_w4(wp + (int64_t)(32 * i) * d);
    }
  };
  auto load_keys = [&]() {
    int C_w, row0_w;
    {
      const int ws = __builtin_amdgcn_readfirstlane(w_row);
      if (ws < 8) { C_w = __builtin_amdgcn_readlane(vC8, ws); row0_w = __builtin_amdgcn_readlane(vR8, ws); }
      else { C_w = gld(a.win_C + ws); row0_w = gld(a.win_row0 + ws); }
    }
    C = min(C_w, CMAX);
    Kh = a.ckv + (int64_t)row0_w * a.ldkv + a.koff + h * 64;
    Vh = Kh + d;
#pragma unroll
    for (int t = 0; t < NTILE; t++)
#pragma unroll
      for (int i = 0; i < SL; i++) {
        const int key = min(t * KT + rg + 32 * i, C - 1);
        kv[t][i] = gld4(Kh + (key * a.ldkv + c4));
      }
  };
  {
    const int c = tid < d ? tid : 0;
    const float* pp = a.pend + (int64_t)r * d + c;
    const int64_t plane = (int64_t)a.S * d;
    if constexpr (PS) {
#if !defined(WB_PS_DRY)
      if (!ps.known_dead) {
        load_weights();
        load_keys();
      }
#endif
      if (!ps_wait(ps)) return false;
      dead = ps.known_dead ? 1 : ld_i<true>(ps.dead + r);
      if (r >= n_live || dead) { ps.saw_dead = true; return true; }
      const Buf16 xgb(a.g_x_in), pgb(a.g_pend);
      const uint32_t pvo = (uint32_t)(r * d + c);
// ... 72 lines not shown
  {
    float acc[4] = {0.f, 0.f, 0.f, 0.f};
    const int q4 = lane >> 4;
#pragma unroll
    for (int i = 0; i < NWQ; i++) {
      const float xv = lane_get(xn_own, 4 * i + q4);
      acc[0] += xv * wqr[i].x; acc[1] += xv * wqr[i].y; acc[2] += xv * wqr[i].z; acc[3] += xv * wqr[i].w;
    }
#pragma unroll
    for (int c = 0; c < 4; c++) { acc[c] = xor16_sum(acc[c]); acc[c] = xor32_sum(acc[c]); }
    if (lane < 16) *reinterpret_cast<float4*>(&red[wave][c4]) = make_float4(acc[0], acc[1], acc[2], acc[3]);
  }
  __syncthreads();
  if constexpr (PS) ps_stamp_fine(ps, 5);
  const int cf = tid % CF, jg = tid / CF;
  const bool p5 = jg < G;
  const int jb = (p5 ? jg : 0) * RPG;
  float4 wo[RPG];
  {
    const float* wp = a.Wo + (int64_t)(h * 64 + jb) * d + cf * 4;
    if (RG::NWO_X == 0 || res == nullptr) {
#pragma unroll
      for (int i = 0; i < RG::NWO_X; i++) wo[i] = ld_w4(wp + (int64_t)i * d);
    }
#pragma unroll
    for (int i = RG::NWO_X; i < RPG; i++) wo[i] = ld_w4(wp + (int64_t)i * d);
  }
  if (tid < 64) {
    float v = 0.f;
#pragma unroll
    for (int w8 = 0; w8 < 8; w8++) v += red[w8][tid];
    qv[tid] = (v + qbias) * a.scale;
  }
  __syncthreads();
  if constexpr (PS) ps_stamp(ps, 3);
  {
    const float4 q4 = *reinterpret_cast<const float4*>(&qv[c4]);
#pragma unroll
    for (int p = 0; p < NP; p++) {
      const float* nxt = p + 1 < NP ? Kh + (p + 1) * PASS_C * a.ldkv : Vh;
      int rgp = rg;
      if constexpr (NP > 1) WB_LAUNDER_V(rgp);
#pragma unroll
      for (int t = 0; t < NTILE; t++) {
        if constexpr (NP > 1) __builtin_amdgcn_sched_barrier(0);
#pragma unroll
        for (int i = 0; i < SL; i++) {
          const int k0 = t * KT + rgp + 32 * i, key = p * PASS_C + k0;
          float s = q4.x * kv[t][i].x + q4.y * kv[t][i].y + q4.z * kv[t][i].z + q4.w * kv[t][i].w;
          s += dpp_f<DPP_QUAD_XOR1, 0xF>(0.f, s);
          s += dpp_f<DPP_QUAD_XOR2, 0xF>(0.f, s);
          s += dpp_f<DPP_ROW_HALF_MIRROR, 0xF>(0.f, s);
          s += dpp_f<DPP_ROW_MIRROR, 0xF>(0.f, s);
          if ((tid & 15) == 0 && key < C) sc[key] = s;
          const int lim = p + 1 < NP ? max(C - 1 - (p + 1) * PASS_C, -(p + 1) * PASS_C) : C - 1;
          if (t >= RG::NVT || !res_v) kv[t][i] = gld4(nxt + (min(k0, lim) * a.ldkv + c4));
        }
      }
    }
  }
  __syncthreads();
  if constexpr (PS) ps_stamp(ps, 4);
  float m = -INFINITY;
  for (int j = lane; j < C; j += 64) m = fmaxf(m, sc[j]);
  m = wave_max(m);
  float l = 0.f;
  for (int j = lane; j < C; j += 64) l += expf(sc[j] - m);
  l = wave_sum(l);
  for (int j = tid; j < C; j += NT) pbuf[j] = expf(sc[j] - m);
  __syncthreads();
  {
    float4 o = make_float4(0.f, 0.f, 0.f, 0.f);
#pragma unroll
    for (int p = 0; p < NP; p++) {
      int rgp = rg;
      if constexpr (NP > 1) WB_LAUNDER_V(rgp);
#pragma unroll
      for (int t = 0; t < NTILE; t++) {
        if constexpr (NP > 1) WB_PIN_F4(o);
#pragma unroll
        for (int i = 0; i < SL; i++) {
          const int k0 = t * KT + rgp + 32 * i, key = p * PASS_C + k0;
          const float pk = key < C ? pbuf[key] : 0.f;
          if (t < RG::NVT) { if (res_v) kv[t][i] = res_ld(res, t * SL + i, tid); }
          o.x += pk * kv[t][i].x; o.y += pk * kv[t][i].y; o.z += pk * kv[t][i].z; o.w += pk * kv[t][i].w;
          if (p + 1 < NP)
            kv[t][i] = gld4(Vh + (min(key + PASS_C, C - 1) * a.ldkv + c4));
        }
      }
    }
    *reinterpret_cast<float4*>(&part[rg][c4]) = o;
  }
  __syncthreads();
  if (tid < 64) {
    float v = 0.f;
#pragma unroll
    for (int g2 = 0; g2 < 32; g2++) v += part[g2][tid];
    att[tid] = v / l;
  }
  __syncthreads();
  if constexpr (PS) ps_stamp(ps, 5);
  if constexpr (RG::NWO_X > 0) {
    if (res != nullptr) {
#pragma unroll
      for (int i = 0; i < RG::NWO_X; i++) wo[i] = res_ld(res, RG::WO_X + i, tid);
    }
  }
  float ov[4] = {0.f, 0.f, 0.f, 0.f};
#pragma unroll
  for (int i = 0; i < RPG; i++) {
    const float av = att[jb + i];
    ov[0] += av * wo[i].x; ov[1] += av * wo[i].y; ov[2] += av * wo[i].z; ov[3] += av * wo[i].w;
  }
  if (p5 && jg > 0) *reinterpret_cast<float4*>(&obuf[(jg - 1) * d + cf * 4]) = make_float4(ov[0], ov[1], ov[2], ov[3]);
  __syncthreads();
  if (jg == 0) {
#pragma unroll
    for (int g2 = 1; g2 < G; g2++) {
      const float4 t = *reinterpret_cast<const float4*>(&obuf[(g2 - 1) * d + cf * 4]);
      ov[0] += t.x; ov[1] += t.y; ov[2] += t.z; ov[3] += t.w;
    }
    if constexpr (PS) {
      const Buf16 pgo(a.g_P);
      st_gran4(pgo, (uint32_t)((h * a.S + r) * d + cf * 4), ps.tag_out, make_float4(ov[0], ov[1], ov[2], ov[3]));
    } else {
      *reinterpret_cast<float4*>(&a.P[((int64_t)h * a.S + r) * d + cf * 4]) = make_float4(ov[0], ov[1], ov[2], ov[3]);
    }
  }
  if (h == 0 && tid < d) {
    if constexpr (PS) { const Buf16 xgo(a.g_x_out); st_gran(xgo, (uint32_t)(r * d + tid), ps.tag_out, xfold); }
    else a.x_out[(int64_t)r * d + tid] = xfold;
  }
  return true;
}

template <int DPL, int NP, int RS>
__device__ __forceinline__ void dec_cross_res_fill(const CrossFusedArgs& a, const int h, const int r, float4* res) {
  using RG = ResGeom<DPL, NP, RS>;
  constexpr int d = 64 * DPL, CF = d / 4, G = RG::G, RPG = RG::RPG, KT = 128, SL = RG::SL;
  const int tid = role_tid<true>();
  const int rg = tid >> 4, c4 = (tid & 15) * 4;
  if constexpr (RG::NVT > 0) {
    const int C = min(gld(a.win_C + r), CROSS_FUSED_MAX_C), row0 = gld(a.win_row0 + r);
    const float* Vh = a.ckv + (int64_t)row0 * a.ldkv + a.koff + h * 64 + d;
#pragma unroll 1
    for (int t = 0; t < RG::NVT; t++) {
      float4 v[SL];
#pragma unroll
      for (int i = 0; i < SL; i++) v[i] = gld4(Vh + (min(t * KT + rg + 32 * i, C - 1) * a.ldkv + c4));
#pragma unroll
      for (int i = 0; i < SL; i++) res_st(res, t * SL + i, tid, v[i]);
    }
  }
  if constexpr (RG::NWO_X > 0) {
    const int cf = tid % CF, jg = tid / CF;
    const int jb = (jg < G ? jg : 0) * RPG;
    const float* wp = a.Wo + (int64_t)(h * 64 + jb) * d + cf * 4;
    float4 w[RG::NWO_X];
#pragma unroll
    for (int i = 0; i < RG::NWO_X; i++) w[i] = ld_w4(wp + (int64_t)i * d);
#pragma unroll
    for (int i = 0; i < RG::NWO_X; i++) res_st(res, RG::WO_X + i, tid, w[i]);
  }
}


}
}
```

### whisper-burn_amd/csrc/decode_persist.hip

```cpp
#include <hip/hip_runtime.h>

#include <climits>
#include <vector>

#include "decode.h"
#include "decode_fused_bodies.h"
#include "handoff.h"
#include "wave_ops.h"

namespace wb {
namespace {

using namespace fused;

constexpr int PS_NT = 512;
constexpr int PS_CT = 128;
constexpr int PS_NGO = 16;

template <int DPL>
struct FinLnLds { alignas(16) float hs[64 * DPL]; };
template <int DPL>
__device__ __forceinline__ bool ps_finln_role(const PersistArgs& a, const int r, const PsStep& ps, FinLnLds<DPL>& sm) {
  constexpr int d = 64 * DPL, FP = 4 * DPL;
  auto& hs = sm.hs;
// ... 298 lines not shown
  const int NL = a.n_layer, S = a.S, R = a.n_rows, H = a.n_head, NB = a.nb_mlp;
  auto cptr = [&](int c) { return reinterpret_cast<unsigned*>(a.ctl + HX_HDR + c * HX_LINE); };
  const int C_X = 0, C_ATTN = S, C_CROSS = S + NL * S, C_MLP = C_CROSS + NL, C_LOG = C_MLP + NL, C_GO = C_LOG + 8;
  int n_per_ctr[8];
#pragma unroll
  for (int k = 0; k < 8; k++) n_per_ctr[k] = (a.n_logits_roles + 7 - k) / 8;
  const int i_lo = a.role_off[blockIdx.x], i_hi = a.role_off[blockIdx.x + 1];
#if defined(WB_PS_DRY)
  constexpr bool RES = false;
#else
  constexpr bool RES = RS > 0;
#endif
  int res_i = -1;
  if (RES && a.res_role != nullptr) res_i = a.res_role[blockIdx.x];
  if (res_i >= i_lo && res_i < i_hi) {
    const PsRole role = a.roles[res_i];
    if (role.kind == PSR_ATTN) dec_attn_res_fill<DPL, RS>(a.layers[role.layer].attn, role.a, res_buf);
    else if (role.kind == PSR_CROSS) dec_cross_res_fill<DPL, NP, RS>(a.layers[role.layer].cross, role.a, role.b, res_buf);
  }
  unsigned long long dead_seen = 0;
  for (int e = 0; e < a.n_steps; e++) {
    for (int i = i_lo; i < i_hi; i++) {
      const PsRole role = a.roles[i];
      PsStep ps;
      ps.known_dead = i - i_lo < 64 && ((dead_seen >> (i - i_lo)) & 1ull) != 0;
      ps.ctl = a.ctl; ps.step = a.step0 + e; ps.n_rows = R; ps.dead = a.dead; ps.lds_flag = &wait_flag[0];
      unsigned long long* stp = a.stamps ? a.stamps + ((size_t)e * a.n_roles + i) * PS_STAMPS : nullptr;
      if (stp && threadIdx.x == 0) stp[0] = wall_clock64();
      ps.stamp = stp;
      int out;
      bool ok;
      const unsigned tag_l = a.tag_base + 2u + 3u * (unsigned)(e * NL + (role.kind <= PSR_MLP ? role.layer : NL - 1));
      if (role.kind == PSR_ATTN) {
        const AttnFusedArgs la = a.layers[role.layer].attn;
        if (role.layer == 0) { ps.ctr_index = C_X + role.b; ps.target = (unsigned)e; }
        else { ps.ctr_index = C_CROSS + role.layer - 1; ps.target = (unsigned)(e + 1) * H * R; }
        ps.ctr = cptr(ps.ctr_index);
        ps.tag_out = tag_l; ps.tag_in = tag_l - 1u;
        ok = dec_attn_body<DPL, true, RS>(la, role.a, role.b, ps, lds.attn, i == res_i ? res_buf : nullptr);
        out = C_ATTN + role.layer * S + role.b;
      } else if (role.kind == PSR_CROSS) {
        const CrossFusedArgs la = a.layers[role.layer].cross;
        if (role.layer == 0) { ps.ctr_index = C_X + role.b; ps.target = (unsigned)e; }
        else { ps.ctr_index = C_MLP + role.layer - 1; ps.target = (unsigned)(e + 1) * NB; }
        ps.ctr = cptr(ps.ctr_index);
        ps.tag_out = tag_l + 1u; ps.tag_in = tag_l;
        ok = dec_cross_body<DPL, true, NP, RS>(la, role.a, role.b, ps, lds.cross, i == res_i ? res_buf : nullptr);
        out = C_CROSS + role.layer;
      } else if (role.kind == PSR_MLP) {
        const MlpFusedArgs la = a.layers[role.layer].mlp;
        ps.ctr_index = C_ATTN + role.layer * S; ps.target = (unsigned)(e + 1) * H; ps.n_ctr = R;
        ps.ctr = cptr(ps.ctr_index);
        ps.tag_out = tag_l + 2u; ps.tag_in = tag_l + 1u;
        ok = dec_mlp_body<MR, DPL, false, true>(la, role.a, ps, lds.mlp);
        out = C_MLP + role.layer;
      } else if (role.kind == PSR_FINLN) {
        ps.ctr_index = C_CROSS + NL - 1; ps.target = (unsigned)(e + 1) * H * R;
        ps.ctr = cptr(ps.ctr_index);
        ps.tag_in = tag_l + 2u; ps.tag_out = tag_l + 2u;
        ok = ps_finln_role<DPL>(a, role.b, ps, lds.finln);
        out = C_GO + PS_NGO;
      } else if (role.kind == PSR_LOGITS) {
        ps.ctr_index = C_GO + (role.layer % PS_NGO); ps.target = (unsigned)(e + 1);
        ps.ctr = cptr(ps.ctr_index);
        ps.tag_in = tag_l + 2u;
        ok = ps_logits_role<MR, DPL>(a, role.a, role.b, ps, e < a.n_forced, lds.logits);
        out = C_LOG + (role.layer & 7);
      } else {
        ok = ps_merge_role(a, role.b, e, ps, cptr(C_LOG), n_per_ctr, lds.merge);
        out = C_X + role.b;
      }
      if (!ok) return;
      if (ps.saw_dead && i - i_lo < 64) dead_seen |= 1ull << (i - i_lo);
      if (stp && threadIdx.x == 0) stp[6] = wall_clock64();
      if (role.kind == PSR_CROSS && role.layer == NL - 1)
        hx_arrive_broadcast(cptr(out), (unsigned)(e + 1) * H * R, cptr(C_GO), PS_NGO, (unsigned)(e + 1));
      else
        hx_arrive(cptr(out));
      if (stp && threadIdx.x == 0) stp[7] = wall_clock64();
    }
  }
}

__global__ void ps_seed_kernel(const float* __restrict__ x, int n, void* gx, unsigned tag) {
  const Buf16 b(gx);
  for (int i = blockIdx.x * blockDim.x + threadIdx.x; i < n; i += gridDim.x * blockDim.x) st_gran(b, (uint32_t)i, tag, x[i]);
}

template <int DPL, int MR, int NP>
int max_blocks_per_cu() {
  int nb = 0;
  if (hipOccupancyMaxActiveBlocksPerMultiprocessor(&nb, (dec_persist_kernel<DPL, MR, NP>), PS_NT, 0) != hipSuccess) return 0;
  return nb;
}

}

int dec_persist_resident_slots(int d, int n_rows, int max_keys) {
  if (!dec_persist_supported(d, n_rows, max_keys)) return 0;
  const int dpl = d / 64, mr = n_rows > 4 ? 8 : 4, np = max_keys > CROSS_FUSED_MAX_C ? 2 : 1;
#define WB_PS_SLOTS(DPL_, MR_, NP_) \
  if (dpl == DPL_ && mr == MR_ && np == NP_) return PsArena<DPL_, MR_, NP_>::USEFUL ? PsArena<DPL_, MR_, NP_>::RS : 0;
  WB_PS_INSTANCES(WB_PS_SLOTS)
#undef WB_PS_SLOTS
  return 0;
}

int ps_ctl_ints(int S, int n_layer) { return HX_HDR + (S + n_layer * S + 2 * n_layer + 8 + PS_NGO + 1) * HX_LINE; }

bool dec_persist_supported(int d, int n_rows, int max_keys) {
  if (n_rows < 1 || n_rows > 8) return false;
  if (max_keys > CROSS_FUSED_MAX_PASSES * CROSS_FUSED_MAX_C) return false;
  if (max_keys > CROSS_FUSED_MAX_C && n_rows > 4) return false;
  if (d == 128 || d == 384) return true;
  return d == 512 && n_rows <= 4;
}

int dec_persist_max_grid(int device, int d, int n_rows, int max_keys) {
  if (!dec_persist_supported(d, n_rows, max_keys)) return 0;
  int cus = 0, coop = 0;
  if (hipDeviceGetAttribute(&coop, hipDeviceAttributeCooperativeLaunch, device) != hipSuccess || !coop) return 0;
  if (hipDeviceGetAttribute(&cus, hipDeviceAttributeMultiprocessorCount, device) != hipSuccess || cus <= 0) return 0;
  int per = 0;
  const bool big = n_rows > 4;
  if (max_keys > CROSS_FUSED_MAX_C)
    per = d == 128 ? max_blocks_per_cu<2, 4, 2>() : d == 384 ? max_blocks_per_cu<6, 4, 2>() : max_blocks_per_cu<8, 4, 2>();
  else if (d == 128) per = big ? max_blocks_per_cu<2, 8, 1>() : max_blocks_per_cu<2, 4, 1>();
  else if (d == 384) per = big ? max_blocks_per_cu<6, 8, 1>() : max_blocks_per_cu<6, 4, 1>();
  else per = max_blocks_per_cu<8, 4, 1>();
  if (per <= 0) return 0;
  return cus * 1;
}

void launch_ps_seed(hipStream_t st, const float* x, int n, void* gx, unsigned tag) {
  hipLaunchKernelGGL(ps_seed_kernel, dim3((n + 255) / 256), dim3(256), 0, st, x, n, gx, tag);
}

int launch_dec_persist(hipStream_t st, const PersistArgs& a, int grid) {
  const dim3 g(grid), b(PS_NT);
  const bool big = a.n_rows > 4;
  hipError_t e = hipErrorInvalidValue;
#define WB_PS(DPL_, MR_, NP_) e = WB_LAUNCH_COOP((dec_persist_kernel<DPL_, MR_, NP_>), g, b, 0, st, a)
  if (a.n_pass > 1) {
    if (big) return -1;
    if (a.d == 128) WB_PS(2, 4, 2); else if (a.d == 384) WB_PS(6, 4, 2); else if (a.d == 512) WB_PS(8, 4, 2);
  }
  else if (a.d == 128) { if (big) WB_PS(2, 8, 1); else WB_PS(2, 4, 1); }
  else if (a.d == 384) { if (big) WB_PS(6, 8, 1); else WB_PS(6, 4, 1); }
  else if (a.d == 512 && !big) WB_PS(8, 4, 1);
#undef WB_PS
  return e == hipSuccess ? 0 : -1;
}

}
```

### whisper-burn_amd/csrc/sample_chain.cpp

```cpp
#include <cmath>
#include <cstring>
#include <limits>

#include "decode_step.h"

using namespace wb;

namespace wb {

int session_sample_chain(wb_session* s, const int32_t* prompt, int P, const SampleCall& sp, const uint8_t* active,
                         const int32_t* stream_ids, int eot, int max_depth, int mask_until_len, int32_t* out_tokens,
                         int32_t row_stride, int32_t* out_lens, double* out_sum, int32_t* out_best) {
  wb_model* m = s->m;
  const wb_dims& D = m->dims;
  const int W = s->W, V = D.n_vocab, bo = sp.best_of;
  WB_REQUIRE(sp.temperature > 0.f && std::isfinite(sp.temperature) && std::isfinite(1.0f / sp.temperature), WB_ERR_ARG,
             "sampling: temperature %g must be finite and > 0, and so must 1 / temperature", (double)sp.temperature);
  WB_REQUIRE(bo >= 1 && bo <= s->max_beams, WB_ERR_ARG, "sampling: best_of %d outside [1, %d]", bo, s->max_beams);
  WB_REQUIRE(P >= 1 && max_depth >= 0, WB_ERR_ARG, "sampling: prompt_len %d / max_depth %d", P, max_depth);
  WB_REQUIRE(row_stride >= P + max_depth, WB_ERR_ARG, "row_stride %d < %d", row_stride, P + max_depth);
  for (int i = 0; i < P; i++) WB_REQUIRE(prompt[i] >= 0 && prompt[i] < V, WB_ERR_ARG, "prompt token %d out of range", prompt[i]);
  WB_REQUIRE(eot >= 0 && eot < V, WB_ERR_ARG, "end-of-text token out of range");
  WB_REQUIRE(sp.attempt >= 0, WB_ERR_ARG, "sampling: attempt %d", sp.attempt);
  WB_REQUIRE(s->step == 0, WB_ERR_STATE, "wb_session_decode_sample: the session is at step %d (wb_session_rewind first)", s->step);
// ... 80 lines not shown
        WB_TRY(launch_step(s, plan, call));
        if (profile().on) profile().ms[4] += run;
        enq += run;
      }
      depth += enq;
      WB_HIP(hipMemcpyAsync(hdr, s->sc_ctl.p, sizeof(hdr), hipMemcpyDeviceToHost, st));
      WB_HIP(hipStreamSynchronize(st));
      if (hdr[SC_ALLDONE] || hdr[SC_ERR]) break;
    }
    tm.stop();
    WB_HIP(hipMemcpyAsync(ctl.data(), s->sc_ctl.p, ctl.size() * 4, hipMemcpyDeviceToHost, st));
    WB_HIP(hipStreamSynchronize(st));
    tm.collect();
    if (profile().on) prof_collect();
    s->prof_step_off = 0;
    for (int r = 0; r < R; r++) steps_done = std::max(steps_done, ctl[sl.ngen + r]);
  }
  s->step += steps_done;
  s->prev_n = 0; s->prev_len.clear(); s->prev_win.clear();
  s->last_had_logits = 0;
  WB_TRY(dec_split_check(s));
  WB_REQUIRE(ctl[SC_ERR] == 0, WB_ERR_STATE, "sampling: a logits row was not finite");
  const double* sum = reinterpret_cast<const double*>(ctl.data() + sl.sum);
  bool all_done = true;
  s->smp_best_of = bo; s->smp_depth = sl.max_depth;
  s->smp_tokens.assign((size_t)W * bo * sl.max_depth, 0);
  s->smp_len.assign((size_t)W * bo, -1);
  for (int a = 0; a < nA; a++) {
    const int w = wa[a];
    int best = 0;
    double best_rank = -INFINITY;
    for (int j = 0; j < bo; j++) {
      const int r = a * bo + j, ng = ctl[sl.ngen + r];
      const int n_text = ng - ((ng > 0 && ctl[sl.tokens + r * sl.max_depth + ng - 1] == eot) ? 1 : 0);
      const double rank = n_text > 0 ? sum[r] / (double)n_text : -INFINITY;
      if (rank > best_rank) { best_rank = rank; best = j; }
      if (out_sum) out_sum[(size_t)w * bo + j] = sum[r];
      s->smp_len[(size_t)w * bo + j] = ng;
      for (int i = 0; i < ng; i++) s->smp_tokens[((size_t)w * bo + j) * sl.max_depth + i] = ctl[sl.tokens + r * sl.max_depth + i];
      all_done = all_done && ctl[sl.fin + r] != 0;
    }
    const int r = a * bo + best, ng = ctl[sl.ngen + r];
    int32_t* row = out_tokens + (size_t)w * row_stride;
    for (int i = 0; i < P; i++) row[i] = prompt[i];
    for (int i = 0; i < ng; i++) row[P + i] = ctl[sl.tokens + r * sl.max_depth + i];
    out_lens[w] = P + ng;
    if (out_best) out_best[w] = best;
  }
  if (max_depth < asked_depth && !all_done)
    WB_REQUIRE(false, WB_ERR_SHAPE, "Token sequence length %d must not exceed %d.", s->Lmax + 1, s->Lmax);
  return WB_OK;
}

}

extern "C" {

void wb_sample_params_default(wb_sample_params* p) {
  if (!p) return;
  p->temperature = 1.0f; p->best_of = 5; p->seed = 0; p->attempt = 0;
}

int wb_session_rewind(wb_session* s) {
  WB_REQUIRE(s, WB_ERR_ARG, "wb_session_rewind: null argument");
  wb::GpuTurn turn(s->device);
  session_rewind(s);
  return WB_OK;
}

int wb_session_last_samples(wb_session* s, int32_t* tokens, int32_t row_stride, int32_t* lens) {
  WB_REQUIRE(s && tokens && lens, WB_ERR_ARG, "wb_session_last_samples: null argument");
  WB_REQUIRE(s->smp_best_of > 0 && (int)s->smp_len.size() == s->W * s->smp_best_of, WB_ERR_STATE,
             "wb_session_last_samples: no sampling call on this session");
  WB_REQUIRE(row_stride >= s->smp_depth, WB_ERR_ARG, "row_stride %d < %d", row_stride, s->smp_depth);
  for (size_t i = 0; i < s->smp_len.size(); i++) {
    lens[i] = s->smp_len[i];
    for (int l = 0; l < s->smp_len[i]; l++) tokens[i * row_stride + l] = s->smp_tokens[i * s->smp_depth + l];
  }
  return WB_OK;
}

int wb_session_graph_count(const wb_session* s) { return s ? (int)s->graphs.size() : 0; }
int64_t wb_session_graph_captures(const wb_session* s) { return s ? s->n_captures : 0; }

int wb_session_decode_sample(wb_session* s, const wb_decode_params* p, const wb_sample_params* sp, const int32_t* prompt,
                             int32_t prompt_len, const uint8_t* active, const int32_t* stream_ids, int32_t* out_tokens,
                             int32_t row_stride, int32_t* out_lens, double* out_sum_logprob, int32_t* out_best) {
  WB_REQUIRE(s && p && sp && prompt && out_tokens && out_lens, WB_ERR_ARG, "wb_session_decode_sample: null argument");
  wb::GpuTurn turn(s->device);
  const SampleCall c{sp->temperature, sp->best_of, sp->seed, sp->attempt};
  return session_sample_chain(s, prompt, prompt_len, c, active, stream_ids, p->tok_end_of_text, p->max_depth, p->mask_until_len,
                              out_tokens, row_stride, out_lens, out_sum_logprob, out_best);
}

int wb_sample_rows(int device, const float* logits, int32_t R, int32_t ld, int32_t V, const float* mask,
                   const uint8_t* row_masked, const float* row_stats, float temperature, uint64_t seed, int32_t attempt,
                   const int32_t* stream, const int32_t* position, int32_t eot, int32_t* out_token, float* out_logprob,
                   int32_t* out_err) {
  WB_REQUIRE(logits && row_stats && stream && position && out_token && out_logprob && out_err, WB_ERR_ARG, "wb_sample_rows: null argument");
  WB_REQUIRE(R >= 1 && V >= 1 && ld >= V && (int64_t)R * ld < ((int64_t)1 << 31), WB_ERR_ARG, "wb_sample_rows: R %d, V %d, ld %d", R, V, ld);
  WB_REQUIRE((mask != nullptr) == (row_masked != nullptr), WB_ERR_ARG, "wb_sample_rows: mask and row_masked go together");
  WB_REQUIRE(temperature > 0.f && std::isfinite(temperature) && std::isfinite(1.0f / temperature), WB_ERR_ARG, "wb_sample_rows: temperature %g", (double)temperature);
  WB_REQUIRE(eot >= 0 && eot < V && attempt >= 0, WB_ERR_ARG, "wb_sample_rows: eot %d / attempt %d", eot, attempt);
  wb::GpuTurn turn(device);
  WB_HIP(hipSetDevice(device));
  DevMem dx, dmask, du8, dst, di32, dout;
  WB_TRY(dx.alloc((size_t)R * ld * 4));
  WB_TRY(dmask.alloc((size_t)V * 4));
  WB_TRY(du8.alloc((size_t)R));
  WB_TRY(dst.alloc((size_t)R * 2 * 4));
  WB_TRY(di32.alloc((size_t)R * 2 * 4));
  constexpr size_t GUARD = 64;
  const size_t out_words = (size_t)2 * R + 1;
  WB_TRY(dout.alloc((out_words + 2 * GUARD) * 4));
  hipStream_t st = nullptr;
  WB_HIP(hipMemsetAsync(dout.p, 0xFF, dout.bytes, st));
  WB_HIP(hipMemcpyAsync(dx.p, logits, (size_t)R * ld * 4, hipMemcpyHostToDevice, st));
  WB_HIP(hipMemcpyAsync(dst.p, row_stats, (size_t)R * 2 * 4, hipMemcpyHostToDevice, st));
  WB_HIP(hipMemcpyAsync(di32.p, stream, (size_t)R * 4, hipMemcpyHostToDevice, st));
  WB_HIP(hipMemcpyAsync(di32.as<int32_t>() + R, position, (size_t)R * 4, hipMemcpyHostToDevice, st));
  if (mask) {
    WB_HIP(hipMemcpyAsync(dmask.p, mask, (size_t)V * 4, hipMemcpyHostToDevice, st));
    WB_HIP(hipMemcpyAsync(du8.p, row_masked, (size_t)R, hipMemcpyHostToDevice, st));
  }
  SampleRowsArgs a;
  a.logits = dx.as<float>(); a.R = R; a.ld = ld; a.V = V;
  a.mask = mask ? dmask.as<float>() : nullptr; a.row_masked = mask ? du8.as<uint8_t>() : nullptr;
  a.row_stats = dst.as<float>();
  a.inv_t = 1.0f / temperature; a.seed_lo = (uint32_t)(seed & 0xffffffffull); a.seed_hi = (uint32_t)(seed >> 32);
  a.attempt = (uint32_t)attempt;
  a.stream = di32.as<int32_t>(); a.position = a.stream + R; a.eot = eot;
  a.out_token = dout.as<int32_t>() + GUARD; a.out_logprob = reinterpret_cast<float*>(a.out_token + R);
  a.out_err = a.out_token + 2 * R;
  WB_HIP(hipMemsetAsync(a.out_err, 0, 4, st));
  prof_tag(KC_SAMPLE_UPDATE, 4.0 * (double)R * V);
  launch_sample_rows(st, a);
  WB_HIP(hipGetLastError());
  WB_HIP(hipMemcpyAsync(out_token, a.out_token, (size_t)R * 4, hipMemcpyDeviceToHost, st));
  WB_HIP(hipMemcpyAsync(out_logprob, a.out_logprob, (size_t)R * 4, hipMemcpyDeviceToHost, st));
  WB_HIP(hipMemcpyAsync(out_err, a.out_err, 4, hipMemcpyDeviceToHost, st));
  uint32_t guards[2][GUARD];
  WB_HIP(hipMemcpyAsync(guards[0], dout.p, GUARD * 4, hipMemcpyDeviceToHost, st));
  WB_HIP(hipMemcpyAsync(guards[1], dout.as<int32_t>() + GUARD + out_words, GUARD * 4, hipMemcpyDeviceToHost, st));
  WB_HIP(hipStreamSynchronize(st));
  for (int b = 0; b < 2; b++)
    for (size_t i = 0; i < GUARD; i++)
      WB_REQUIRE(guards[b][i] == 0xFFFFFFFFu, WB_ERR_STATE, "wb_sample_rows: guard band %d overwritten at word %zu", b, i);
  return WB_OK;
}

}
```

### whisper-burn_amd/csrc/session.cpp

```cpp
#include "session.h"

#include <cstring>
#include <mutex>

#include "switches.h"

using namespace wb;

namespace wb {

static std::mutex g_pool_mu;
static std::unordered_map<uint64_t, std::vector<wb_session*>> g_pool;
static uint64_t g_next_model_uid = 1;
constexpr size_t POOL_MAX_SESSIONS = 8;
constexpr size_t POOL_MAX_BYTES = (size_t)4 << 30;

void session_pool_register(wb_model* m) {
  std::lock_guard<std::mutex> lk(g_pool_mu);
  m->uid = g_next_model_uid++;
  g_pool[m->uid];
}

void session_pool_purge(wb_model* m) {
  std::vector<wb_session*> dead;
// ... 177 lines not shown
    launch_mel_frontend(s->st, fe, pcm_dev, s->wins.as<MelWindow>(), s->W, maxF, s->mel.as<float>(), (int64_t)80 * Ts, Ts,
                        s->gmax.as<float>(), s->padding, Ts, [&]() {
                          if (trace_extra & 2) enc_trace_stage(s->st, "mel0", s->mel.p, (size_t)s->W * 80 * Ts * 4);
                          if (trace_extra & 4)
                            enc_trace_stage(s->st, "gmax", s->gmax.p, (size_t)s->W * mel_bmax_stride(maxF) * 2 * 4);
                        });
    tm.stop();
    if (tm.on) { WB_HIP(hipStreamSynchronize(s->st)); tm.collect(); profile().ms[5] += 1; }
  }
  WB_HIP(hipGetLastError());
  MelBatch mb;
  mb.mel = s->mel.as<float>(); mb.win_stride = (int64_t)80 * Ts; mb.row_stride = Ts; mb.T = s->T;
  return session_finish_encode(s, mb, defer_guard);
}

int session_reserve(wb_session* s, int max_len) {
  wb_model* m = s->m;
  const wb_dims& D = m->dims;
  const int d = D.n_text_state, NL = D.n_text_layer, V = D.n_vocab, S = s->S;
  WB_REQUIRE(d <= 1280, WB_ERR_SHAPE, "decode kernels keep whole rows in LDS: n_state %d > 1280", d);
  WB_REQUIRE(d % 64 == 0, WB_ERR_SHAPE, "decode kernels need n_state %% 64 == 0 (head size 64), got %d", d);
  max_len = std::max(8, std::min(max_len, std::min(D.n_text_ctx, 448)));
  s->Lmax = max_len;
  const size_t pool = (size_t)max_len * S;
  WB_TRY(s->kc.ensure_zeroed((size_t)NL * pool * d * 4, s->st));
  WB_TRY(s->vc.ensure_zeroed((size_t)NL * pool * d * 4, s->st));
  WB_TRY(s->tabs.ensure((size_t)2 * S * max_len * 4));
  s->lay = make_step_layout(S, s->W);
  WB_TRY(s->state.ensure((size_t)s->lay.total * 4));
  const size_t host_bytes = (size_t)s->lay.total * 4 + (size_t)S * TOPK_MAX * 8 + (size_t)S * 2 * 4;
  if (s->host_bytes < host_bytes) {
    if (s->host_block) { (void)hipHostFree(s->host_block); s->host_block = nullptr; s->host_bytes = 0; }
    WB_HIP(hipHostMalloc((void**)&s->host_block, host_bytes, hipHostMallocMapped));
    s->host_bytes = host_bytes;
  }
  WB_HIP(hipHostGetDevicePointer((void**)&s->host_block_dev, s->host_block, 0));
  s->state_host = reinterpret_cast<int*>(s->host_block);
  s->topk_id_host = reinterpret_cast<int32_t*>(s->host_block + (size_t)s->lay.total * 4);
  s->topk_lp_host = reinterpret_cast<float*>(s->host_block + (size_t)s->lay.total * 4 + (size_t)S * TOPK_MAX * 4);
  s->chain_flags_off = (size_t)s->lay.total * 4 + (size_t)S * TOPK_MAX * 8;
  gemv_plan(d, 3 * d, &s->ks_qkv, &s->ksl_qkv);
  gemv_plan(d, d, &s->ks_o, &s->ksl_o);
  gemv_plan(d, 4 * d, &s->ks_1, &s->ksl_1);
  gemv_plan(4 * d, d, &s->ks_2, &s->ksl_2);
  s->ks_v = 1; s->ksl_v = d;
  s->ct_v = GV_CT_LOGITS;
  s->n_tiles_v = (V + s->ct_v - 1) / s->ct_v;
  WB_TRY(s->x.ensure(((size_t)2 * S + 8) * d * 4));
  WB_TRY(s->h.ensure((size_t)S * d * 4));
  WB_TRY(s->att.ensure((size_t)S * d * 4));
  WB_TRY(s->hm.ensure((size_t)S * 4 * d * 4));
  s->sk_qkv = skinny_ksplit(d, 3 * d, KS_MAX, S); s->sk_o = skinny_ksplit(d, d, KS_MAX, S);
  s->sk_1 = skinny_ksplit(d, 4 * d, KS_MAX, S); s->sk_2 = skinny_ksplit(4 * d, d, KS_MAX, S);
  WB_TRY(s->Pqkv.ensure((size_t)std::max(s->ks_qkv, s->sk_qkv) * S * 3 * d * 4));
  WB_TRY(s->Po.ensure(((size_t)std::max(s->ks_o, s->sk_o) * S + 8) * d * 4));
  WB_TRY(s->Pq.ensure((size_t)std::max(s->ks_o, s->sk_o) * S * d * 4));
  WB_TRY(s->P1.ensure((size_t)std::max(s->ks_1, s->sk_1) * S * 4 * d * 4));
  WB_TRY(s->P2.ensure(((size_t)std::max(std::max(s->ks_2, s->sk_2), dec_mlp_fused_planes(d)) * S + 8) * d * 4));

  WB_TRY(s->Pa.ensure(((size_t)D.n_text_head * S + 8) * d * 4));
  WB_TRY(s->Pc.ensure(((size_t)D.n_text_head * S + 8) * d * 4));
  WB_TRY(s->carec.ensure(((size_t)D.n_text_head * std::max(1, s->n_chunks) * S + 8) * (d + 2) * 4));
  WB_TRY(s->ca.ensure((size_t)S * D.n_text_head * std::max(1, s->n_chunks) * CA_STRIDE * 4));
  WB_TRY(s->logits.ensure((size_t)S * V * 4));
  WB_TRY(s->tstats.ensure((size_t)S * s->n_tiles_v * TS_STRIDE * 4));
  WB_TRY(s->row_stats.ensure((size_t)S * 2 * 4));
  WB_TRY(s->lp_tmp.ensure((size_t)V * 4));
  s->decode_ready = true;
  return WB_OK;
}

}

void wb_session::clear_graphs() {
  for (auto& kv : graphs) (void)hipGraphExecDestroy(kv.second);
  graphs.clear();
}

wb_session::~wb_session() {
  clear_graphs();
  if (host_block) (void)hipHostFree(host_block);
  if (guard_host) (void)hipHostFree(guard_host);
  if (pcm_stage) (void)hipHostFree(pcm_stage);
  if (ev_seg) (void)hipEventDestroy(ev_seg);
  if (st2) (void)hipStreamDestroy(st2);
  if (st) (void)hipStreamDestroy(st);
}

extern "C" {

int wb_session_begin(wb_model* m, const float* pcm, int64_t n_pcm, const int64_t* starts, const int64_t* lens,
                     int n_windows, int max_beams, int padding, wb_session** out) {
  WB_REQUIRE(m && pcm && starts && lens && out, WB_ERR_ARG, "wb_session_begin: null argument");
  wb::GpuTurn turn(m->device);
  wb_session* s = nullptr;
  WB_TRY(session_create(m, n_windows, max_beams, padding, &s));
  int rc = session_encode_pcm(s, pcm, n_pcm, starts, lens, false);
  if (rc != WB_OK) { wb_session_free(s); return rc; }
  *out = s;
  return WB_OK;
}

int wb_session_begin_mel(wb_model* m, const float* mel, const int32_t* T, int n_windows, int max_beams, int padding,
                         wb_session** out) {
  WB_REQUIRE(m && mel && T && out, WB_ERR_ARG, "wb_session_begin_mel: null argument");
  wb::GpuTurn turn(m->device);
  wb_session* s = nullptr;
  WB_TRY(session_create(m, n_windows, max_beams, padding, &s));
  const int clip = m->max_mel_frames() - padding;
  int maxT = 0;
  for (int w = 0; w < n_windows; w++) {
    if (T[w] < 1) { wb_session_free(s); set_error("window %d: empty mel", w); return WB_ERR_SHAPE; }
    s->T[w] = std::min(T[w], clip) + padding;
    maxT = std::max(maxT, s->T[w]);
  }
  const int Ts = (maxT + 3) & ~3;
  std::vector<float> host((size_t)n_windows * 80 * Ts, 0.f);
  const float* src = mel;
  for (int w = 0; w < n_windows; w++) {
    const int keep = s->T[w] - padding;
    for (int r = 0; r < 80; r++) memcpy(&host[((size_t)w * 80 + r) * Ts], src + (size_t)r * T[w], (size_t)keep * 4);
    src += (size_t)80 * T[w];
  }
  int rc = s->mel.ensure(host.size() * 4);
  if (rc == WB_OK && (hipMemcpyAsync(s->mel.p, host.data(), host.size() * 4, hipMemcpyHostToDevice, s->st) != hipSuccess ||
                      hipStreamSynchronize(s->st) != hipSuccess)) {
    set_error("mel upload failed");
    rc = WB_ERR_HIP;
  }
  if (rc == WB_OK) {
    MelBatch mb;
    mb.mel = s->mel.as<float>(); mb.win_stride = (int64_t)80 * Ts; mb.row_stride = Ts; mb.T = s->T;
    rc = session_finish_encode(s, mb);
  }
  if (rc != WB_OK) { wb_session_free(s); return rc; }
  *out = s;
  return WB_OK;
}

void wb_session_free(wb_session* s) {
  if (!s) return;
  {
    std::lock_guard<std::mutex> lk(g_pool_mu);
    auto it = g_pool.find(s->model_uid);
    if (it != g_pool.end()) {
      size_t parked = 0;
      for (const wb_session* q : it->second) parked += session_device_bytes(q);
      if (sw::session_pool() && it->second.size() < POOL_MAX_SESSIONS && parked + session_device_bytes(s) <= POOL_MAX_BYTES) {
        it->second.push_back(s);
        return;
      }
    }
  }
  (void)hipSetDevice(s->device);
  delete s;
}

int wb_session_set_special_mask(wb_session* s, const uint8_t* is_special) {
  WB_REQUIRE(s && is_special, WB_ERR_ARG, "wb_session_set_special_mask: null argument");
  wb::GpuTurn turn(s->device);
  const int V = s->m->dims.n_vocab;
  WB_HIP(hipSetDevice(s->m->device));
  WB_TRY(s->mask.ensure((size_t)V * 4));
  if (s->mask_dev_ptr == s->mask.p && (int)s->mask_host.size() == V && memcmp(s->mask_host.data(), is_special, (size_t)V) == 0) {
    s->has_mask = true;
    return WB_OK;
// ... 42 lines not shown
```

### whisper-burn_amd/csrc/session.h

```cpp
#pragma once
#include <vector>

#include "decode.h"
#include "engine.h"

struct wb_session {
  wb_model* m = nullptr;
  uint64_t model_uid = 0;
  int device = 0;
  hipStream_t st = nullptr;
  hipStream_t st2 = nullptr;
  hipEvent_t ev_seg = nullptr;
  int W = 0, max_beams = 0, S = 0, padding = 0;
  double sample_rate = 16000.0;
  int Lmax = 0;
  std::vector<int> T, C, row0;
  std::vector<wb::MelWindow> wins_host; void* wins_dev_ptr = nullptr;
  std::vector<int> meta_host; void* meta_dev_ptr = nullptr;
  std::vector<uint8_t> mask_host; void* mask_dev_ptr = nullptr;
  int enc_rows = 0, maxC = 0, n_chunks = 0;
  wb::Workspace ws;
  wb::DevMem pcm, mel, wins, gmax, enc_out, ckv, win_meta;
  float* pcm_stage = nullptr; size_t pcm_stage_bytes = 0;
  wb::DevMem kc, vc, tabs, state;
  wb::StepLayout lay;
  char* host_block = nullptr;
  char* host_block_dev = nullptr;
  size_t host_bytes = 0;
  size_t chain_flags_off = 0;
  int* state_host = nullptr;
  int32_t* topk_id_host = nullptr;
  float* topk_lp_host = nullptr;
  wb::DevMem x, h, att, Pqkv, Po, Pq, P1, P2, Pa, Pc, carec, ca, logits, tstats, row_stats, mask, lp_tmp, gctl, gtok, hm;
  int sk_qkv = 0, sk_o = 0, sk_1 = 0, sk_2 = 0;
  wb::DevMem ps_layers, ps_roles, ps_ctl, ps_dead, ps_tstats, ps_stamps;
  wb::DevMem ps_gx, ps_gpa, ps_gpc, ps_gp2, ps_gxn;
  unsigned ps_launches = 0;
  int ps_grid = -1;
  int n_tiles_v = 0, ct_v = 128;
  int ks_qkv = 1, ksl_qkv = 0, ks_o = 1, ksl_o = 0, ks_1 = 1, ksl_1 = 0, ks_2 = 1, ksl_2 = 0, ks_v = 1, ksl_v = 0;
  wb::DevMem bc_ctl, bc_topk;
  wb::DevMem sc_ctl, sc_topk;
  uint64_t sample_sig = 0;
  std::vector<int32_t> smp_tokens, smp_len; int smp_best_of = 0, smp_depth = 0;
  std::vector<int> prev_len, prev_win;
  int prev_n = 0, step = 0;
  bool has_mask = false, decode_ready = false;
  int last_use_mask = 0, last_had_logits = 0;
  int prof_cls_cross = -1, prof_cls_self = -1, prof_step_off = 0;
  int* guard_host = nullptr; int* guard_dev = nullptr;
  bool enc_guard_pending = false;
  wb::MelBatch enc_mb;
  std::unordered_map<uint64_t, hipGraphExec_t> graphs;
  int64_t n_captures = 0;
  uint64_t buf_sig = 0;
  uint64_t beam_sig = 0;
  void clear_graphs();
  ~wb_session();
};

namespace wb {
struct Profile {
  bool on = false;
  double ms[8] = {0, 0, 0, 0, 0, 0, 0, 0};
};
Profile& profile();
struct KernelStat { int64_t calls = 0; double ms = 0, bytes = 0; };
void prof_adjust_bytes(int cls, double delta);
void prof_collect();
struct ScopedTimer {
  hipStream_t st; int slot; hipEvent_t a = nullptr, b = nullptr; bool on;
  ScopedTimer(hipStream_t s, int slot_);
  void stop();
  void collect();
  ~ScopedTimer();
};

void session_pool_register(wb_model* m);
void session_pool_purge(wb_model* m);
int session_create(wb_model* m, int n_windows, int max_beams, int padding, wb_session** out);
int session_encode_pcm(wb_session* s, const float* pcm, int64_t n_pcm, const int64_t* starts, const int64_t* lens,
                       bool pcm_on_device, bool defer_guard = false);
int session_enc_guard_resolve(wb_session* s, bool* reencoded);
void session_rewind(wb_session* s);
int session_reserve(wb_session* s, int max_len);
int session_beam_chain(wb_session* s, const int32_t* prompt, int prompt_len, int beam_size, int eot, int max_depth,
                       int mask_until_len, int32_t* out_tokens, int32_t row_stride, int32_t* out_lens, bool* handled);
struct SampleCall { float temperature; int best_of; uint64_t seed; int attempt; };
int session_sample_chain(wb_session* s, const int32_t* prompt, int prompt_len, const SampleCall& sp, const uint8_t* active,
                         const int32_t* stream_ids, int eot, int max_depth, int mask_until_len, int32_t* out_tokens,
                         int32_t row_stride, int32_t* out_lens, double* out_sum, int32_t* out_best);
int session_greedy_chain(wb_session* s, const int32_t* prompt, int eot, int max_depth, int mask_until_len, int prompt_len,
                         int32_t* out_tokens, int32_t row_stride, int32_t* out_lens);
int session_align(wb_session* s, const int32_t* tokens, int32_t row_stride, const int32_t* lens, const int32_t* heads,
                  int32_t n_heads, int32_t n_prefix, int32_t drop_last, int32_t filter_width, int32_t* start_pos,
                  float* matrix, const int32_t* drop_last_rows);
int session_score(wb_session* s, const int32_t* tokens, int32_t row_stride, const int32_t* lens, int32_t mask_until_len,
                  const int32_t* probe_ids, int32_t n_probe, int32_t probe_pos, float* token_logprobs,
                  float* probe_logprobs);
}
```

### whisper-burn_amd/csrc/switches.h

```cpp
#pragma once

namespace wb {
namespace sw {

enum Kind { DEFAULT_ON, OPT_IN, UNSET_OR_1, TRI, INT, STR };

#define WB_BOOL_SWITCHES(X)                                                                                                          \
  X(graph, "WHISPER_HIP_GRAPH", DEFAULT_ON, "on", "replay captured hipGraphs of the decode steps; 0: enqueue every step eagerly")    \
  X(chain, "WHISPER_HIP_CHAIN", DEFAULT_ON, "on", "device-chained greedy decode; 0: one host round trip per step")                   \
  X(beam_chain, "WHISPER_HIP_BEAM_CHAIN", DEFAULT_ON, "on", "beam bookkeeping on the device; 0: host-driven beam search")            \
  X(persist, "WHISPER_HIP_PERSIST", DEFAULT_ON, "on", "persistent flag-chained greedy kernel; 0: one launch per sublayer")           \
  X(persist_prefill, "WHISPER_HIP_PERSIST_PREFILL", DEFAULT_ON, "on", "the persistent launch runs the prompt itself; 0: host prefill") \
  X(poll, "WHISPER_HIP_POLL", DEFAULT_ON, "on", "chained greedy: spin on mapped progress flags; 0: copy + synchronise per chunk")    \
  X(speculate, "WHISPER_HIP_SPECULATE", OPT_IN, "off", "chained greedy: enqueue one segment ahead of the finished flags")            \
  X(fuse_sub, "WHISPER_HIP_FUSE_SUB", DEFAULT_ON, "on", "fused self-attention and MLP sublayer kernels; 0: per-matrix GEMVs")        \
  X(fuse_x, "WHISPER_HIP_FUSE_X", DEFAULT_ON, "on", "fused cross-attention sublayer kernel; 0: chunked cross-attention + GEMV")      \
  X(fuse_q, "WHISPER_HIP_FUSE_Q", DEFAULT_ON, "on", "chunked cross-attention blocks project their own queries")                      \
  X(fuse_co, "WHISPER_HIP_FUSE_CO", OPT_IN, "off", "chunked cross-attention blocks apply the out-projection too")                    \
  X(fuse16, "WHISPER_HIP_FUSE16", DEFAULT_ON, "on", "9 - 16 live rows stay on the fused sublayer kernels; 0: batch mode")            \
  X(batch_skinny, "WHISPER_HIP_BATCH_SKINNY", DEFAULT_ON, "on", "batch mode: skinny weight-stream GEMM up to 64 rows; 0: tiled GEMM") \
  X(cross_stream, "WHISPER_HIP_CROSS_STREAM", DEFAULT_ON, "on", "batch mode, one beam per window: streaming cross-attention")        \
  X(sk_pair, "WHISPER_HIP_SK_PAIR", OPT_IN, "off", "skinny GEMM: the waves' partial tiles meet pairwise")                            \
  X(mlp16_mfma, "WHISPER_HIP_MLP16_MFMA", DEFAULT_ON, "on", "9 - 16-row fused MLP on the matrix cores; 0: two row groups of 8")      \
  X(logits_mfma, "WHISPER_HIP_LOGITS_MFMA", DEFAULT_ON, "on", "9 - 16-row logits product on the matrix cores")                       \
  X(logits_preln, "WHISPER_HIP_LOGITS_PRELN", DEFAULT_ON, "on", "9 - 16-row logits: fold + LayerNorm once, in its own launch")       \
  X(logits_mr16, "WHISPER_HIP_LOGITS_MR16", DEFAULT_ON, "on", "9 - 16-row logits GEMV as one 16-row tile")                           \
  X(encoder_split, "WHISPER_HIP_ENCODER_SPLIT", UNSET_OR_1, "on", "split-precision (fp16 hi / lo) encoder-side GEMMs; 0: exact f32") \
  X(decoder_split, "WHISPER_HIP_DECODER_SPLIT", DEFAULT_ON, "on", "split-precision batch-mode decoder GEMM; 0: exact f32")           \
  X(encoder_pieces, "WHISPER_HIP_ENCODER_PIECES", DEFAULT_ON, "on", "encoder activations travel as fp16 pieces between split GEMMs") \
  X(attn_f16, "WHISPER_HIP_ATTN_F16", DEFAULT_ON, "on", "encoder attention on fp16 pieces; 0: the f32 kernels")                      \
  X(attn_kvsplit, "WHISPER_HIP_ATTN_KVSPLIT", DEFAULT_ON, "on", "encoder attention splits long key ranges across blocks")            \
  X(gpu_turn, "WHISPER_HIP_GPU_TURN", DEFAULT_ON, "on", "one entry point at a time per device and process (developer: 0 drops it)")  \
  X(session_pool, "WHISPER_HIP_SESSION_POOL", DEFAULT_ON, "on", "released sessions are parked for reuse; 0: freed (developer A/B)")  \
  X(pcm_stage, "WHISPER_HIP_PCM_STAGE", OPT_IN, "off", "host PCM is uploaded through a pinned per-session buffer")
#define WB_INT_SWITCHES(X)                                                                                                           \
  X(cross_stream_fuse, "WHISPER_HIP_CROSS_STREAM_FUSE", TRI, -1, "streaming cross-attention folds / projects its query; unset: d <= 768") \
  X(sk_max_blocks, "WHISPER_HIP_SK_MAX_BLOCKS", INT, 256, "skinny GEMM: most blocks a K-split may launch")                           \
  X(split_tile, "WHISPER_HIP_SPLIT_TILE", INT, 0, "split-precision GEMM: force a tile shape (developer A/B; 0: choose)")             \
  X(enc_trace_extra, "WHISPER_HIP_ENC_TRACE_EXTRA", INT, 0, "bit mask of extra stages in the encoder trace (1 pcm, 2 mel, 4 maxima)")
#define WB_STR_SWITCHES(X)                                                                                                           \
  X(enc_trace, "WHISPER_HIP_ENC_TRACE", STR, nullptr, "directory for per-thread dumps of the encoder stages (developer)")            \
  X(ps_stamps, "WHISPER_HIP_PS_STAMPS", STR, nullptr, "file for the persistent kernel's role timeline (developer)")                  \
  X(persist_resident, "WHISPER_HIP_PERSIST_RESIDENT", STR, nullptr, "persistent kernel: step-invariant operands stay in LDS (on); 0: off; log: on + report") \
  X(persist_inject_fail, "WHISPER_HIP_PERSIST_INJECT_FAIL", STR, nullptr, "test hook: \"launch\" = the cooperative launch is refused")

#define WB_SW_DECL(fn, name, kind, dflt, what) bool fn();
WB_BOOL_SWITCHES(WB_SW_DECL)
#undef WB_SW_DECL
#define WB_SW_DECL(fn, name, kind, dflt, what) int fn();
WB_INT_SWITCHES(WB_SW_DECL)
#undef WB_SW_DECL
#define WB_SW_DECL(fn, name, kind, dflt, what) const char* fn();
WB_STR_SWITCHES(WB_SW_DECL)
#undef WB_SW_DECL

}
}
```

### whisper-burn_amd/whisper_burn_amd/_lib.py

```python
from __future__ import annotations

import ctypes as C
import os

_HERE = os.path.dirname(os.path.abspath(__file__))
LIB_PATH = os.path.join(os.path.dirname(_HERE), "lib", "libwhisper_hip.so")

c_float_p = C.POINTER(C.c_float)
c_int32_p = C.POINTER(C.c_int32)
c_int64_p = C.POINTER(C.c_int64)
c_uint8_p = C.POINTER(C.c_uint8)
c_double_p = C.POINTER(C.c_double)


class WbDims(C.Structure):
    _fields_ = [(n, C.c_int32) for n in (
        "n_mels", "n_audio_ctx", "n_audio_state", "n_audio_head", "n_audio_layer",
        "n_vocab", "n_text_ctx", "n_text_state", "n_text_head", "n_text_layer")]


class WbDecodeParams(C.Structure):
    _fields_ = [(n, C.c_int32) for n in (
        "beam_size", "max_depth", "padding", "overlap_seconds", "max_n_offsets", "min_n_overlaps",
        "mask_until_len", "max_batch_windows",
# ... 41 lines not shown
    "wb_wav_read_f32": (C.c_int, [C.c_char_p, c_float_p, C.c_int64, c_int64_p]),
    "wb_wav_read_f32_any_rate": (C.c_int, [C.c_char_p, c_float_p, C.c_int64, c_int64_p]),
    "wb_resample_len": (C.c_int64, [C.c_int64, C.c_int32, C.c_int32]),
    "wb_resample_filter": (C.c_int, [C.c_int32, C.c_int32, c_float_p, C.c_int32, c_int32_p, c_int32_p, c_int32_p]),
    "wb_resample_dev": (C.c_int, [C.c_int, C.c_void_p, C.c_int64, C.c_int32, C.c_int32, C.c_void_p, C.c_int64, c_int64_p]),
    "wb_pcm_s16_to_f32_dev": (C.c_int, [C.c_int, C.c_void_p, C.c_int64, C.c_void_p]),
    "wb_waveform_to_mels_dev": (C.c_int, [C.c_int, C.c_void_p, C.c_int64, C.c_double, c_int64_p, c_int64_p, C.c_int32,
                                          C.c_int32, C.c_int32, C.c_void_p, C.c_int64, C.c_int32, c_int32_p, C.c_int32,
                                          c_double_p]),
    "wb_waveform_to_mels_dev_frontend": (C.c_int, [C.c_int, C.c_void_p, C.c_int64, C.c_double, c_int64_p, c_int64_p,
                                                   C.c_int32, C.c_int32, C.c_int32, C.c_void_p, C.c_int64, C.c_int32,
                                                   c_int32_p, C.c_int32, c_double_p, C.c_int32]),
    "wb_forward_encoder": (C.c_int, [C.c_void_p, c_float_p, C.c_int, C.c_int, c_float_p]),
    "wb_forward_decoder": (C.c_int, [C.c_void_p, c_int32_p, C.c_int, C.c_int, c_float_p, C.c_int, c_float_p]),
    "wb_forward": (C.c_int, [C.c_void_p, c_float_p, C.c_int, C.c_int, c_int32_p, C.c_int, c_float_p]),
    "wb_decode_params_default": (None, [C.POINTER(WbDecodeParams)]),
    "wb_comm_unique_id": (C.c_int, [c_uint8_p]),
    "wb_comm_init": (C.c_int, [c_uint8_p, C.c_int, C.c_int, C.c_int, C.POINTER(C.c_void_p)]),
    "wb_comm_free": (None, [C.c_void_p]),
    "wb_comm_allgather": (C.c_int, [C.c_void_p, C.c_void_p, C.c_void_p, C.c_int64]),
    "wb_shard_partition": (C.c_int, [C.c_int64, C.c_int, C.c_int, c_int64_p, c_int64_p]),
    "wb_waveform_to_tokens_sharded": (C.c_int, [C.c_void_p, C.c_void_p, C.c_int, C.c_int64, C.c_int, C.POINTER(WbDecodeParams),
                                               c_uint8_p, C.c_int, C.c_int, C.c_void_p, C.c_void_p, c_int32_p, C.c_int32,
                                               c_int32_p, C.c_int64, c_int32_p, C.c_int64, c_int64_p]),
    "wb_session_begin": (C.c_int, [C.c_void_p, c_float_p, C.c_int64, c_int64_p, c_int64_p, C.c_int, C.c_int,
                                   C.c_int, C.POINTER(C.c_void_p)]),
    "wb_session_begin_mel": (C.c_int, [C.c_void_p, c_float_p, c_int32_p, C.c_int, C.c_int, C.c_int,
                                       C.POINTER(C.c_void_p)]),
    "wb_session_set_special_mask": (C.c_int, [C.c_void_p, c_uint8_p]),
    "wb_session_step": (C.c_int, [C.c_void_p, c_int32_p, c_int32_p, c_int32_p, C.c_int, C.c_int, C.c_int,
                                  c_int32_p, c_float_p]),
    "wb_session_last_logprobs": (C.c_int, [C.c_void_p, C.c_int, c_float_p]),
    "wb_session_encoder_output": (C.c_int, [C.c_void_p, C.c_int, c_float_p, c_int32_p]),
    "wb_session_free": (None, [C.c_void_p]),
    "wb_session_decode": (C.c_int, [C.c_void_p, C.POINTER(WbDecodeParams), c_int32_p, C.c_int32, c_int32_p]),
    "wb_session_decode_prompt": (C.c_int, [C.c_void_p, C.POINTER(WbDecodeParams), c_int32_p, C.c_int32, c_int32_p, C.c_int32,
                                           c_int32_p]),
    "wb_waveform_to_tokens_prompted": (C.c_int, [C.c_void_p, c_float_p, C.c_int64, C.c_int, C.POINTER(WbDecodeParams),
                                                 c_uint8_p, C.c_int32, C.c_int32, c_int32_p, C.c_int32, c_int32_p,
                                                 c_int32_p, C.c_int64, c_int64_p]),
    "wb_beam_search_device": (C.c_int, [C.c_int, C.POINTER(WbDecodeParams), C.c_int, C.c_int, C.c_void_p, C.c_void_p, c_int32_p,
                                        C.c_int32, c_int32_p]),
    "wb_beam_search": (C.c_int, [C.POINTER(WbDecodeParams), C.c_int, C.c_int, C.c_void_p, C.c_void_p, c_int32_p,
                                 C.c_int32, c_int32_p]),
    "wb_waveform_to_tokens": (C.c_int, [C.c_void_p, c_float_p, C.c_int64, C.c_int, C.POINTER(WbDecodeParams),
                                        c_uint8_p, C.c_int, C.c_int, c_int32_p, C.c_int32, c_int32_p,
                                        c_int32_p, C.c_int64, c_int64_p]),
    "wb_waveform_to_tokens_dev": (C.c_int, [C.c_void_p, C.c_void_p, C.c_int64, C.c_int, C.POINTER(WbDecodeParams),
                                            c_uint8_p, C.c_int, C.c_int, c_int32_p, C.c_int32, c_int32_p,
                                            c_int32_p, C.c_int64, c_int64_p]),
    "wb_window_extents": (C.c_int64, [C.c_int64, C.c_int, C.c_int64, C.c_int, c_int64_p, c_int64_p, C.c_int64]),
    "wb_find_chunk_overlap": (C.c_int, [c_int32_p, C.c_int64, c_int32_p, C.c_int64, C.c_int, C.c_int,
                                        c_int64_p, c_int64_p]),
    "wb_stitch_windows": (C.c_int, [c_int32_p, C.c_int32, c_int32_p, C.c_int, C.c_int, C.c_int, c_int32_p,
                                    C.c_int64, c_int64_p]),
    "wb_align_tokens": (C.c_int, [C.c_void_p, c_int32_p, C.c_int, C.c_int, c_int32_p, c_float_p, C.c_int, c_int32_p,
                                  C.c_int32, C.c_int32, C.c_int32, C.c_int32, c_int32_p, c_float_p]),
    "wb_session_align": (C.c_int, [C.c_void_p, c_int32_p, C.c_int32, c_int32_p, c_int32_p, C.c_int32, C.c_int32,
                                   C.c_int32, C.c_int32, c_int32_p, c_float_p]),
    "wb_dtw_start_positions": (C.c_int, [C.c_int, c_float_p, C.c_int32, C.c_int32, c_int32_p]),
    "wb_waveform_to_token_times": (C.c_int, [C.c_void_p, c_float_p, C.c_int64, C.c_int, C.POINTER(WbDecodeParams),
                                             c_uint8_p, C.c_int, C.c_int, c_int32_p, C.c_int32, c_int32_p,
                                             c_int32_p, C.c_int64, c_int64_p, c_int32_p, C.c_int32, C.c_int32,
                                             c_float_p, c_float_p]),
    "wb_stitch_windows_times": (C.c_int, [c_int32_p, C.c_int32, c_int32_p, C.c_int, C.c_int, C.c_int, c_int32_p,
                                          C.c_int64, c_int64_p, c_float_p, c_float_p]),
    "wb_score_tokens": (C.c_int, [C.c_void_p, c_int32_p, C.c_int, C.c_int, c_int32_p, c_float_p, C.c_int, c_uint8_p,
                                  C.c_int32, c_int32_p, C.c_int32, C.c_int32, c_float_p, c_float_p]),
    "wb_session_score": (C.c_int, [C.c_void_p, c_int32_p, C.c_int32, c_int32_p, C.c_int32, c_int32_p, C.c_int32,
                                   C.c_int32, c_float_p, c_float_p]),
    "wb_waveform_detect_language": (C.c_int, [C.c_void_p, c_float_p, C.c_int64, C.c_int, C.c_int32, C.c_int32, c_int32_p,
                                              C.c_int32, C.c_int32, c_float_p, c_float_p, c_int32_p]),
    "wb_waveform_to_token_scores": (C.c_int, [C.c_void_p, c_float_p, C.c_int64, C.c_int, C.POINTER(WbDecodeParams),
                                              c_uint8_p, C.c_int, C.c_int, c_int32_p, C.c_int32, c_int32_p,
                                              c_int32_p, C.c_int64, c_int64_p, C.c_int32, c_float_p, c_float_p,
                                              c_float_p, c_float_p]),
    "wb_logprob_gather": (C.c_int, [C.c_int, c_float_p, C.c_int32, C.c_int32, c_float_p, C.c_int32, c_float_p, c_uint8_p,
                                    c_int32_p, c_int32_p, c_int32_p, C.c_int32, C.c_int32, c_float_p, c_float_p,
                                    c_float_p]),
    "wb_sample_params_default": (None, [C.POINTER(WbSampleParams)]),
    "wb_session_rewind": (C.c_int, [C.c_void_p]),
    "wb_session_graph_count": (C.c_int, [C.c_void_p]),
    "wb_session_graph_captures": (C.c_int64, [C.c_void_p]),
    "wb_session_decode_sample": (C.c_int, [C.c_void_p, C.POINTER(WbDecodeParams), C.POINTER(WbSampleParams), c_int32_p,
                                           C.c_int32, c_uint8_p, c_int32_p, c_int32_p, C.c_int32, c_int32_p, c_double_p,
                                           c_int32_p]),
    "wb_session_last_samples": (C.c_int, [C.c_void_p, c_int32_p, C.c_int32, c_int32_p]),
    "wb_fallback_params_default": (None, [C.POINTER(WbFallbackParams)]),
    "wb_fallback_decide": (C.c_int, [C.POINTER(WbFallbackParams), C.c_float, C.c_float, C.c_float]),
    "wb_waveform_to_tokens_fallback": (C.c_int, [C.c_void_p, c_float_p, C.c_int64, C.c_int, C.POINTER(WbDecodeParams),
                                                 c_uint8_p, C.c_int, C.c_int, c_int32_p, C.c_int32, c_int32_p,
                                                 c_int32_p, C.c_int64, c_int64_p, C.POINTER(WbFallbackParams), C.c_void_p,
                                                 C.c_void_p, c_float_p, c_int32_p, c_float_p, c_float_p, c_float_p,
                                                 c_int32_p]),
    "wb_sample_rows": (C.c_int, [C.c_int, c_float_p, C.c_int32, C.c_int32, C.c_int32, c_float_p, c_uint8_p, c_float_p,
                                 C.c_float, C.c_uint64, C.c_int32, c_int32_p, c_int32_p, C.c_int32, c_int32_p, c_float_p,
                                 c_int32_p]),
    "wb_first_repetition_end": (C.c_int64, [c_int32_p, C.c_int64, C.c_int64]),
    "wb_repetition_period": (C.c_int64, [c_int32_p, C.c_int64, C.c_int64]),
    "wb_find_repeated_tokens_index": (C.c_int, [c_int32_p, C.c_int64, C.c_int64, C.c_int64, c_int64_p, c_int64_p]),
    "wb_mel_constants": (C.c_int, [C.c_double, c_float_p, c_float_p]),
    "wb_mel_dft_table": (C.c_int, [c_float_p]),
    "wb_profile_enable": (C.c_int, [C.c_int]),
    "wb_profile_read": (C.c_int, [c_double_p, C.c_int]),
    "wb_profile_kernels": (C.c_int, [C.c_void_p, C.c_int, C.c_int]),
    "wb_last_error": (C.c_char_p, []),
    "wb_version": (C.c_char_p, []),
}



class WbKernelStat(C.Structure):
    _fields_ = [("name", C.c_char * 96), ("calls", C.c_int64), ("total_ms", C.c_double), ("algo_bytes", C.c_double)]


def profile_kernels(reset: bool = True):
    lib = load()
    buf = (WbKernelStat * 32)()
    n = min(32, int(lib.wb_profile_kernels(C.cast(buf, C.c_void_p), 32, int(reset))))
    return [dict(name=buf[i].name.decode(), calls=int(buf[i].calls), total_ms=float(buf[i].total_ms),
                 algo_bytes=float(buf[i].algo_bytes)) for i in range(n)]


_lib = None


def load(path: str | None = None) -> C.CDLL:
    global _lib
    if _lib is not None and path is None:
        return _lib
    path = path or os.environ.get("WHISPER_HIP_LIB", LIB_PATH)
    if not os.path.exists(path):
        raise OSError(f"{path} not found: build it with `python -c 'import __graft_entry__ as g; g.build()'` "
                      f"(make -C whisper-burn_amd/csrc); there is no CPU fallback")
    try:
        import torch
    except Exception:
        pass
    lib = C.CDLL(path, mode=C.RTLD_GLOBAL)
    for name, (res, args) in SIGNATURES.items():
        fn = getattr(lib, name)
        fn.restype = res
        fn.argtypes = args
    if b"hipemu" in lib.wb_version() and os.environ.get("WHISPER_HIP_ALLOW_EMU") != "1":
        raise OSError(f"{path} is the hipemu functional-model build, not the gfx950 library; the engine has no CPU "
                      f"path (tests that drive the emulator set WHISPER_HIP_ALLOW_EMU=1)")
    _lib = lib
    return lib


class WbError(RuntimeError):
    def __init__(self, status: int, msg: str):
        super().__init__(f"whisper_hip status {status}: {msg}")
        self.status = status


def check(status: int) -> None:
    if status != 0:
        raise WbError(status, (load().wb_last_error() or b"").decode("utf-8", "replace"))
```

Before: 2241 x real-time.

## Cache persistent-decode launch setup on session and use pinned async control transfers

Builds the persistent kernel's layer args, role tables and resident-role map once per session and reuses them on later calls when a key of shapes and buffer pointers matches. The per-call host-to-device control upload becomes a memset plus a device-side write of the stop flag in the seed kernel, which also removes a stream synchronize before launch. Readback of the error flag, control block and tokens goes through one pinned host buffer with async copies. The resident LDS layout indexing is also reworked, and a geometry query API is added. This trims host-side launch overhead, but risks stale-cache bugs if the key misses some state.

```diff
diff --git a/include/whisper_hip.h b/include/whisper_hip.h
--- a/include/whisper_hip.h
+++ b/include/whisper_hip.h
@@ -225,6 +225,7 @@
 int wb_session_rewind(wb_session* s);
 int wb_session_graph_count(const wb_session* s);
 int64_t wb_session_graph_captures(const wb_session* s);
+int wb_persist_resident_geometry(int32_t n_state, int32_t n_rows, int32_t max_keys, int32_t* out5);
 int wb_session_decode_sample(wb_session* s, const wb_decode_params* p, const wb_sample_params* sp, const int32_t* prompt,
                              int32_t prompt_len, const uint8_t* active, const int32_t* stream_ids, int32_t* out_tokens,
                              int32_t row_stride, int32_t* out_lens, double* out_sum_logprob, int32_t* out_best);
diff --git a/rust/whisper-hip/src/ffi.rs b/rust/whisper-hip/src/ffi.rs
--- a/rust/whisper-hip/src/ffi.rs
+++ b/rust/whisper-hip/src/ffi.rs
@@ -149,6 +149,7 @@
     pub fn wb_session_rewind(s: *mut wb_session) -> c_int;
     pub fn wb_session_graph_count(s: *const wb_session) -> c_int;
     pub fn wb_session_graph_captures(s: *const wb_session) -> i64;
+    pub fn wb_persist_resident_geometry(n_state: i32, n_rows: i32, max_keys: i32, out5: *mut i32) -> c_int;
     pub fn wb_session_last_samples(s: *mut wb_session, tokens: *mut i32, row_stride: i32, lens: *mut i32) -> c_int;
     pub fn wb_sample_rows(device: c_int, logits: *const c_float, R: i32, ld: i32, V: i32, mask: *const c_float,
                           row_masked: *const u8, row_stats: *const c_float, temperature: c_float, seed: u64, attempt: i32,
diff --git a/whisper-burn_amd/csrc/decode.h b/whisper-burn_amd/csrc/decode.h
--- a/whisper-burn_amd/csrc/decode.h
+++ b/whisper-burn_amd/csrc/decode.h
@@ -259,9 +259,10 @@
 int ps_ctl_ints(int S, int n_layer);
 bool dec_persist_supported(int d, int n_rows, int max_keys);
 int dec_persist_resident_slots(int d, int n_rows, int max_keys);
+bool dec_persist_resident_geometry(int d, int n_rows, int max_keys, int out[5]);
 int dec_persist_max_grid(int device, int d, int n_rows, int max_keys);
 int launch_dec_persist(hipStream_t st, const PersistArgs& a, int grid);
-void launch_ps_seed(hipStream_t st, const float* x, int n, void* gx, unsigned tag);
+void launch_ps_seed(hipStream_t st, const float* x, int n, void* gx, unsigned tag, int* ctl);
 
 #if defined(HIPEMU) && !defined(HIPEMU_PROD_GEOMETRY)
 constexpr int CROSS_FUSED_MAX_C = 384;
diff --git a/whisper-burn_amd/csrc/decode_chain.cpp b/whisper-burn_amd/csrc/decode_chain.cpp
--- a/whisper-burn_amd/csrc/decode_chain.cpp
+++ b/whisper-burn_amd/csrc/decode_chain.cpp
@@ -9,11 +9,23 @@
 
 namespace wb {
 
-static int run_persistent_chain(wb_session* s, int eot, int max_depth, int mask_until_len, const int32_t* forced, int n_forced,
-                                int* steps_done, bool* fell_back) {
-  *fell_back = false;
-  WB_REQUIRE(n_forced >= 0 && n_forced <= PS_MAX_FORCED, WB_ERR_ARG, "persistent decode: %d prompt steps", n_forced);
-  const char* inject = sw::persist_inject_fail();
+struct PsPin { size_t seed, err, gctl, tok, total, ctl_ints; };
+static PsPin ps_pin_layout(size_t ctl_ints, size_t tok_ints) {
+  PsPin p;
+  p.seed = 0; p.err = (ctl_ints + 3) & ~(size_t)3; p.gctl = p.err + 4; p.tok = p.gctl + ((ctl_ints + 3) & ~(size_t)3);
+  p.total = p.tok + tok_ints; p.ctl_ints = ctl_ints;
+  return p;
+}
+static int ps_pin_ensure(wb_session* s, size_t ints) {
+  if (s->ps_pin_ints >= ints) return WB_OK;
+  if (s->ps_pin_busy) { WB_HIP(hipStreamSynchronize(s->st)); s->ps_pin_busy = false; }
+  if (s->ps_pin) { (void)hipHostFree(s->ps_pin); s->ps_pin = nullptr; s->ps_pin_ints = 0; }
+  WB_HIP(hipHostMalloc((void**)&s->ps_pin, ints * 4, hipHostMallocDefault));
+  s->ps_pin_ints = ints;
+  return WB_OK;
+}
+
+static int ps_setup_ensure(wb_session* s, bool res_on, bool* built) {
   wb_model* m = s->m;
   const wb_dims& D = m->dims;
   const int d = D.n_text_state, H = D.n_text_head, NL = D.n_text_layer, V = D.n_vocab, S = s->S, W = s->W;
@@ -23,17 +35,21 @@
   const int n_tiles = (V + 127) / 128;
   const size_t pool = (size_t)s->Lmax * S;
   const int ldkv = 2 * d;
-  WB_REQUIRE(NB <= 32 && H <= 8, WB_ERR_SHAPE, "persistent decode: more planes than its folds hold");
-  WB_TRY(s->ps_gx.ensure_zeroed(((size_t)2 * S + 8) * d * 8, st));
-  WB_TRY(s->ps_gpa.ensure_zeroed(((size_t)H * S + 8) * d * 8, st));
-  WB_TRY(s->ps_gpc.ensure_zeroed(((size_t)H * S + 8) * d * 8, st));
-  WB_TRY(s->ps_gp2.ensure_zeroed(((size_t)NB * S + 8) * d * 8, st));
-  WB_TRY(s->ps_gxn.ensure_zeroed(((size_t)S + 8) * d * 8, st));
-  if (((s->ps_launches + 1) & 0xffffu) == 0) {
-    for (DevMem* b : {&s->ps_gx, &s->ps_gpa, &s->ps_gpc, &s->ps_gp2, &s->ps_gxn}) WB_HIP(hipMemsetAsync(b->p, 0, b->bytes, st));
-    s->ps_launches++;
-  }
-  const unsigned tag_base = ((++s->ps_launches) & 0xffffu) << 16;
+  const int n_pass = s->maxC > CROSS_FUSED_MAX_C ? 2 : 1;
+  const int n_layer_roles = NL * (2 * W * H + NB);
+  const int grid = std::max(1, std::min(s->ps_grid, n_layer_roles + n_tiles + 2 * W));
+  auto up = [](const void* p) { return (uint64_t)reinterpret_cast<uintptr_t>(p); };
+  const std::vector<uint64_t> key = {
+      s->model_uid, (uint64_t)W, (uint64_t)S, (uint64_t)s->Lmax, (uint64_t)grid, (uint64_t)n_tiles, (uint64_t)n_pass,
+      (uint64_t)s->enc_rows, (uint64_t)res_on, (uint64_t)m->ln_eps_inside_sqrt, up(s->state.p), up(s->x.p), up(s->P2.p),
+      up(s->Pa.p), up(s->Pc.p), up(s->kc.p), up(s->vc.p), up(s->tabs.p), up(s->ckv.p), up(s->win_meta.p), up(s->ps_gx.p),
+      up(s->ps_gpa.p), up(s->ps_gpc.p), up(s->ps_gp2.p), up(s->ps_gxn.p)};
+  const char* sw_setup = sw::persist_setup();
+  const bool cache_on = !(sw_setup && sw_setup[0] == '0');
+  *built = !(cache_on && !s->ps_setup_key.empty() && s->ps_setup_key == key);
+  if (sw_setup && strstr(sw_setup, "log")) fprintf(stderr, "persist setup: %s\n", *built ? "built" : "reused");
+  if (!*built) return WB_OK;
+  s->ps_setup_key.clear();
   char* gxb[2] = {static_cast<char*>(s->ps_gx.p), static_cast<char*>(s->ps_gx.p) + (size_t)S * d * 8};
   std::vector<PsLayerArgs> la(NL);
   float* xb[2] = {s->x.as<float>(), s->x.as<float>() + (size_t)S * d};
@@ -58,7 +74,7 @@
     ca.ckv = s->ckv.as<float>() + (size_t)l * s->enc_rows * 2 * d; ca.ldkv = ldkv; ca.koff = 0;
     ca.win_row0 = s->win_meta.as<int>(); ca.win_C = s->win_meta.as<int>() + W;
     ca.Wo = b.cout.w; ca.P = s->Pc.as<float>();
-    ca.n_pass = s->maxC > CROSS_FUSED_MAX_C ? 2 : 1;
+    ca.n_pass = n_pass;
     ca.g_x_in = gxb[xi]; ca.g_pend = s->ps_gpa.p; ca.g_x_out = gxb[xi ^ 1]; ca.g_P = s->ps_gpc.p;
     xi ^= 1;
     MlpFusedArgs& ma = la[l].mlp;
@@ -75,7 +91,6 @@
     for (int r = 0; r < W; r++) for (int h = 0; h < H; h++) lr.push_back(PsRole{PSR_CROSS, l, h, r});
     for (int j = 0; j < NB; j++) lr.push_back(PsRole{PSR_MLP, l, j, 0});
   }
-  const int grid = std::max(1, std::min(s->ps_grid, (int)lr.size() + n_tiles + 2 * W));
   std::vector<std::vector<PsRole>> deal(grid);
   for (size_t i = 0; i < lr.size(); i++) deal[i % grid].push_back(lr[i]);
   std::vector<int> cand;
@@ -111,46 +126,80 @@
     roles.insert(roles.end(), deal[b].begin(), deal[b].end());
   }
   role_off[grid] = (int)roles.size();
-  const char* res_sw = sw::persist_resident();
-  const bool res_on = !(res_sw && res_sw[0] == '0') && dec_persist_resident_slots(d, W, s->maxC) > 0;
   std::vector<int> res_role(grid, -1);
   int n_res = 0;
   if (res_on)
     for (int b = 0; b < grid; b++) {
-      int n_layer_roles = 0, at = -1;
+      int n_lr = 0, at = -1;
       for (int i = role_off[b]; i < role_off[b + 1]; i++)
-        if (roles[i].kind <= PSR_MLP) { n_layer_roles++; at = i; }
-      if (n_layer_roles == 1 && roles[at].kind != PSR_MLP) { res_role[b] = at; n_res++; }
-    }
+        if (roles[i].kind <= PSR_MLP) { n_lr++; at = i; }
+      if (n_lr == 1 && roles[at].kind != PSR_MLP) { res_role[b] = at; n_res++; }
+    }
+  WB_TRY(s->ps_layers.ensure(la.size() * sizeof(PsLayerArgs)));
+  WB_TRY(s->ps_roles.ensure(roles.size() * sizeof(PsRole) + (role_off.size() + res_role.size()) * 4));
+  WB_HIP(hipMemcpyAsync(s->ps_layers.p, la.data(), la.size() * sizeof(PsLayerArgs), hipMemcpyHostToDevice, st));
+  WB_HIP(hipMemcpyAsync(s->ps_roles.p, roles.data(), roles.size() * sizeof(PsRole), hipMemcpyHostToDevice, st));
+  WB_HIP(hipMemcpyAsync(static_cast<char*>(s->ps_roles.p) + roles.size() * sizeof(PsRole), role_off.data(), role_off.size() * 4,
+                        hipMemcpyHostToDevice, st));
+  WB_HIP(hipMemcpyAsync(static_cast<char*>(s->ps_roles.p) + roles.size() * sizeof(PsRole) + role_off.size() * 4, res_role.data(),
+                        res_role.size() * 4, hipMemcpyHostToDevice, st));
+  WB_HIP(hipStreamSynchronize(st));
+  s->ps_pin_busy = false;
+  s->ps_roles_host.swap(roles);
+  s->ps_setup_grid = grid; s->ps_setup_n_lg = n_lg; s->ps_setup_n_res = n_res;
+  s->ps_setup_key = key;
+  return WB_OK;
+}
+
+static int run_persistent_chain(wb_session* s, int eot, int max_depth, int mask_until_len, const int32_t* forced, int n_forced,
+                                const PsPin& pin, int* steps_done, bool* fell_back) {
+  *fell_back = false;
+  WB_REQUIRE(n_forced >= 0 && n_forced <= PS_MAX_FORCED, WB_ERR_ARG, "persistent decode: %d prompt steps", n_forced);
+  const char* inject = sw::persist_inject_fail();
+  wb_model* m = s->m;
+  const wb_dims& D = m->dims;
+  const int d = D.n_text_state, H = D.n_text_head, NL = D.n_text_layer, V = D.n_vocab, S = s->S, W = s->W;
+  const StepLayout& L = s->lay;
+  hipStream_t st = s->st;
+  const int NB = dec_mlp_fused_planes(d);
+  const int n_tiles = (V + 127) / 128;
+  WB_REQUIRE(NB <= 32 && H <= 8, WB_ERR_SHAPE, "persistent decode: more planes than its folds hold");
+  WB_TRY(s->ps_gx.ensure_zeroed(((size_t)2 * S + 8) * d * 8, st));
+  WB_TRY(s->ps_gpa.ensure_zeroed(((size_t)H * S + 8) * d * 8, st));
+  WB_TRY(s->ps_gpc.ensure_zeroed(((size_t)H * S + 8) * d * 8, st));
+  WB_TRY(s->ps_gp2.ensure_zeroed(((size_t)NB * S + 8) * d * 8, st));
+  WB_TRY(s->ps_gxn.ensure_zeroed(((size_t)S + 8) * d * 8, st));
+  if (((s->ps_launches + 1) & 0xffffu) == 0) {
+    for (DevMem* b : {&s->ps_gx, &s->ps_gpa, &s->ps_gpc, &s->ps_gp2, &s->ps_gxn}) WB_HIP(hipMemsetAsync(b->p, 0, b->bytes, st));
+    s->ps_launches++;
+  }
+  const unsigned tag_base = ((++s->ps_launches) & 0xffffu) << 16;
+  char* gxb[2] = {static_cast<char*>(s->ps_gx.p), static_cast<char*>(s->ps_gx.p) + (size_t)S * d * 8};
+  const char* res_sw = sw::persist_resident();
+  const bool res_on = !(res_sw && res_sw[0] == '0') && dec_persist_resident_slots(d, W, s->maxC) > 0;
+  bool built = false;
+  WB_TRY(ps_setup_ensure(s, res_on, &built));
+  const std::vector<PsRole>& roles = s->ps_roles_host;
+  const int grid = s->ps_setup_grid, n_res = s->ps_setup_n_res;
   if (res_sw && !strcmp(res_sw, "log")) fprintf(stderr, "persist resident blocks: %d of %d\n", n_res, grid);
   const int n_ctl = ps_ctl_ints(S, NL);
-  WB_TRY(s->ps_layers.ensure(la.size() * sizeof(PsLayerArgs)));
-  WB_TRY(s->ps_roles.ensure(roles.size() * sizeof(PsRole) + (role_off.size() + res_role.size()) * 4));
   WB_TRY(s->ps_ctl.ensure((size_t)n_ctl * 4));
   WB_TRY(s->ps_dead.ensure((size_t)S * 4));
   WB_TRY(s->ps_tstats.ensure((size_t)S * n_tiles * 2 * 4));
-  std::vector<int> ctl0(n_ctl, 0);
-  ctl0[HX_STOP] = INT_MAX;
-  WB_HIP(hipMemcpyAsync(s->ps_layers.p, la.data(), la.size() * sizeof(PsLayerArgs), hipMemcpyHostToDevice, st));
-  WB_HIP(hipMemcpyAsync(s->ps_roles.p, roles.data(), roles.size() * sizeof(PsRole), hipMemcpyHostToDevice, st));
-  WB_HIP(hipMemcpyAsync(static_cast<char*>(s->ps_roles.p) + roles.size() * sizeof(PsRole) + role_off.size() * 4, res_role.data(),
-                        res_role.size() * 4, hipMemcpyHostToDevice, st));
-  WB_HIP(hipMemcpyAsync(static_cast<char*>(s->ps_roles.p) + roles.size() * sizeof(PsRole), role_off.data(), role_off.size() * 4,
-                        hipMemcpyHostToDevice, st));
-  WB_HIP(hipMemcpyAsync(s->ps_ctl.p, ctl0.data(), (size_t)n_ctl * 4, hipMemcpyHostToDevice, st));
+  WB_HIP(hipMemsetAsync(s->ps_ctl.p, 0, (size_t)n_ctl * 4, st));
   WB_HIP(hipMemsetAsync(s->ps_dead.p, 0, (size_t)S * 4, st));
   PersistArgs a;
   a.layers = s->ps_layers.as<PsLayerArgs>(); a.roles = s->ps_roles.as<PsRole>(); a.n_roles = (int)roles.size();
   a.role_off = reinterpret_cast<const int*>(static_cast<char*>(s->ps_roles.p) + roles.size() * sizeof(PsRole));
-  if (n_res > 0) a.res_role = a.role_off + role_off.size();
-  a.n_logits_roles = n_lg;
+  if (n_res > 0) a.res_role = a.role_off + (grid + 1);
+  a.n_logits_roles = s->ps_setup_n_lg;
   a.n_layer = NL; a.n_rows = W; a.S = S; a.d = d; a.n_head = H; a.nb_mlp = NB;
   a.n_pass = s->maxC > CROSS_FUSED_MAX_C ? 2 : 1;
   a.ctl = s->ps_ctl.as<int>(); a.step0 = s->step; a.n_steps = n_forced + max_depth; a.mask_until_len = mask_until_len;
   a.n_forced = n_forced;
   for (int i = 0; i < n_forced; i++) a.forced[i] = forced[i];
   a.g_xn = s->ps_gxn.p;
-  a.x_fin = gxb[xi]; a.P2 = s->ps_gp2.p; a.b2_last = m->dec[NL - 1].mlp2.b; a.tag_base = tag_base;
+  a.x_fin = gxb[(3 * NL) & 1]; a.P2 = s->ps_gp2.p; a.b2_last = m->dec[NL - 1].mlp2.b; a.tag_base = tag_base;
   a.ln_g = m->ln_dec.g; a.ln_b = m->ln_dec.b; a.ln_eps = m->ln_dec.eps; a.ln_inside = m->ln_eps_inside_sqrt;
   a.Et = m->tok_emb_t; a.vocab_ld = m->vocab_ld; a.V = V; a.mask = s->mask.as<float>();
   a.tstats = s->ps_tstats.as<float>(); a.n_tiles = n_tiles;
@@ -167,8 +216,7 @@
              "persistent decode: %d layers x %d steps do not fit the 16-bit granule tags", NL, max_depth);
   launch_dec_prepare(st, reinterpret_cast<const int*>(s->host_block_dev), s->state.as<int>(), L, W, s->tabs.as<int>(),
                      s->Lmax, m->tok_emb, m->dec_pos, d, s->x.as<float>(), s->gctl.as<int>());
-  launch_ps_seed(st, s->x.as<float>(), W * d, gxb[0], tag_base + 1u);
-  WB_HIP(hipStreamSynchronize(st));
+  launch_ps_seed(st, s->x.as<float>(), W * d, gxb[0], tag_base + 1u, s->ps_ctl.as<int>());
   hipEvent_t e0 = nullptr, e1 = nullptr;
   prof_tag(KC_PERSIST, 0.0);
   const bool timed = prof_take_events(&e0, &e1);
@@ -182,18 +230,21 @@
     *steps_done = 0;
     return WB_OK;
   }
-  std::vector<int> ctl(n_ctl);
-  WB_HIP(hipMemcpyAsync(ctl.data(), s->ps_ctl.p, (size_t)n_ctl * 4, hipMemcpyDeviceToHost, st));
-  int gstep = 0;
-  WB_HIP(hipMemcpyAsync(&gstep, s->gctl.as<int>() + GC_STEP, 4, hipMemcpyDeviceToHost, st));
+  int* hp = s->ps_pin;
+  s->ps_pin_busy = true;
+  WB_HIP(hipMemcpyAsync(hp + pin.err, s->ps_ctl.as<int>() + HX_ERR, 4, hipMemcpyDeviceToHost, st));
+  WB_HIP(hipMemcpyAsync(hp + pin.gctl, s->gctl.p, pin.ctl_ints * 4, hipMemcpyDeviceToHost, st));
+  WB_HIP(hipMemcpyAsync(hp + pin.tok, s->gtok.p, (pin.total - pin.tok) * 4, hipMemcpyDeviceToHost, st));
   WB_HIP(hipStreamSynchronize(st));
-  if (ctl[HX_ERR] != 0 && gstep == s->step) {
+  s->ps_pin_busy = false;
+  const int err = hp[pin.err], gstep = hp[pin.gctl + GC_STEP];
+  if (err != 0 && gstep == s->step) {
     s->ps_grid = 0;
     *fell_back = true;
     *steps_done = 0;
     return WB_OK;
   }
-  WB_REQUIRE(ctl[HX_ERR] == 0, WB_ERR_HIP, "persistent decode: a wait gave up (counter %d) at step %d", ctl[HX_ERR] - 1, gstep);
+  WB_REQUIRE(err == 0, WB_ERR_HIP, "persistent decode: a wait gave up (counter %d) at step %d", err - 1, gstep);
   if (n_stamps) {
     std::vector<unsigned long long> hs(n_stamps);
     WB_HIP(hipMemcpy(hs.data(), s->ps_stamps.p, n_stamps * 8, hipMemcpyDeviceToHost));
@@ -240,12 +291,17 @@
   WB_TRY(s->gctl.ensure(ctl_ints * 4));
   WB_TRY(s->gtok.ensure(((size_t)S * s->Lmax + 1) * 4));
   std::vector<int> ctl(ctl_ints, 0);
-  auto seed_ctl = [&]() -> int {
-    std::fill(ctl.begin(), ctl.end(), 0);
-    ctl[GC_STEP] = s->step;
-    for (int i = 0; i < W; i++) ctl[GC_HDR + i] = prompt[s->step];
-    WB_HIP(hipMemcpyAsync(s->gctl.p, ctl.data(), ctl_ints * 4, hipMemcpyHostToDevice, st));
-    WB_HIP(hipStreamSynchronize(st));
+  const PsPin pin = ps_pin_layout(ctl_ints, (size_t)S * s->Lmax + 1);
+  WB_TRY(ps_pin_ensure(s, pin.total));
+  auto seed_ctl = [&](bool wait) -> int {
+    if (s->ps_pin_busy) { WB_HIP(hipStreamSynchronize(st)); s->ps_pin_busy = false; }
+    int* seed = s->ps_pin + pin.seed;
+    std::fill(seed, seed + ctl_ints, 0);
+    seed[GC_STEP] = s->step;
+    for (int i = 0; i < W; i++) seed[GC_HDR + i] = prompt[s->step];
+    s->ps_pin_busy = true;
+    WB_HIP(hipMemcpyAsync(s->gctl.p, seed, ctl_ints * 4, hipMemcpyHostToDevice, st));
+    if (wait) { WB_HIP(hipStreamSynchronize(st)); s->ps_pin_busy = false; }
     return WB_OK;
   };
   const StepPlan plan = plan_step(s, W, false);
@@ -261,16 +317,16 @@
   int n_forced = 0;
   if (persist && sw::persist_prefill() && s->step == 0 && n_forced_max <= PS_MAX_FORCED && s->has_mask) n_forced = n_forced_max;
   if (n_forced == 0) WB_TRY(host_prefill());
-  WB_TRY(seed_ctl());
+  WB_TRY(seed_ctl(!persist));
   ScopedTimer tm(st, 3);
   if (persist) {
     bool fell_back = false;
-    WB_TRY(run_persistent_chain(s, eot, max_depth, mask_until_len, prompt + s->step + 1, n_forced, &depth, &fell_back));
+    WB_TRY(run_persistent_chain(s, eot, max_depth, mask_until_len, prompt + s->step + 1, n_forced, pin, &depth, &fell_back));
     if (fell_back) {
       persist = false;
       depth = 0;
       WB_TRY(host_prefill());
-      WB_TRY(seed_ctl());
+      WB_TRY(seed_ctl(true));
       n_forced = 0;
     } else {
       if (profile().on) profile().ms[4] += depth;
@@ -383,10 +439,18 @@
   }
   }
   tm.stop();
-  std::vector<int> toks((size_t)S * s->Lmax + 1);
-  WB_HIP(hipMemcpyAsync(ctl.data(), s->gctl.p, ctl_ints * 4, hipMemcpyDeviceToHost, st));
-  WB_HIP(hipMemcpyAsync(toks.data(), s->gtok.p, toks.size() * 4, hipMemcpyDeviceToHost, st));
-  WB_HIP(hipStreamSynchronize(st));
+  std::vector<int> toks_chain;
+  const int* toks = s->ps_pin + pin.tok;
+  if (persist) {
+    std::copy(s->ps_pin + pin.gctl, s->ps_pin + pin.gctl + ctl_ints, ctl.begin());
+  } else {
+    toks_chain.resize((size_t)S * s->Lmax + 1);
+    WB_HIP(hipMemcpyAsync(ctl.data(), s->gctl.p, ctl_ints * 4, hipMemcpyDeviceToHost, st));
+    WB_HIP(hipMemcpyAsync(toks_chain.data(), s->gtok.p, toks_chain.size() * 4, hipMemcpyDeviceToHost, st));
+    WB_HIP(hipStreamSynchronize(st));
+    s->ps_pin_busy = false;
+    toks = toks_chain.data();
+  }
   tm.collect();
   WB_TRY(dec_split_check(s));
   WB_REQUIRE(ctl[GC_BAD] == 0, WB_ERR_STATE, "a decode step produced a row without a finite log-prob (NaN logits: non-finite "
diff --git a/whisper-burn_amd/csrc/decode_fused_bodies.h b/whisper-burn_amd/csrc/decode_fused_bodies.h
--- a/whisper-burn_amd/csrc/decode_fused_bodies.h
+++ b/whisper-burn_amd/csrc/decode_fused_bodies.h
@@ -118,17 +118,24 @@
 struct ResGeom {
   static constexpr int d = 64 * DPL, G = d / 4 <= 32 ? 8 : 4, RPG = 64 / G;
   static constexpr int KW = d / 8, RK = DPL >= 6 ? 8 : 16, NIT = KW / RK;
-  static constexpr int NRND = (NIT - 2 < RS / RK ? NIT - 2 : RS / RK) > 0 ? (NIT - 2 < RS / RK ? NIT - 2 : RS / RK) : 0;
-  static constexpr int WO_A = NRND * RK;
-  static constexpr int NWO_A = RS - WO_A < RPG ? RS - WO_A : RPG;
+  static constexpr int CAP = RS * ROLE_NT;
+  static constexpr int QL = 8 * 48;
+  static constexpr int WL = G * (d / 4) < ROLE_NT ? G * (d / 4) : ROLE_NT;
+  static constexpr int NRND_MAX = DPL == 6 ? 2 : 1;
+  static constexpr int NRND_FIT = CAP / (RK * QL) < NIT - 2 ? CAP / (RK * QL) : NIT - 2;
+  static constexpr int NRND = NRND_FIT <= 0 ? 0 : (NRND_FIT < NRND_MAX ? NRND_FIT : NRND_MAX);
+  static constexpr int WO_A = NRND * RK * QL;
+  static constexpr int NWO_A = (CAP - WO_A) / WL < RPG ? (CAP - WO_A) / WL : RPG;
   static constexpr int SL = 4, NTILE = CROSS_FUSED_MAX_C / 128;
   static constexpr int NVT = NP > 1 ? 0 : (RS / SL < NTILE ? RS / SL : NTILE);
-  static constexpr int WO_X = NVT * SL;
-  static constexpr int NWO_X = NP > 1 ? 0 : (RS - WO_X < RPG ? RS - WO_X : RPG);
-  static_assert(RS >= 0 && WO_A + NWO_A <= RS && WO_X + NWO_X <= RS, "resident slots");
+  static constexpr int WO_X = NVT * SL * ROLE_NT;
+  static constexpr int NWO_X = NP > 1 ? 0 : ((CAP - WO_X) / WL < RPG ? (CAP - WO_X) / WL : RPG);
+  static_assert(RS >= 0 && WO_A + NWO_A * WL <= CAP && WO_X + NWO_X * WL <= CAP, "resident region");
+  static __device__ __forceinline__ int q_holder(int wave, int lane) { return wave * 48 + (lane < 47 ? lane : 47); }
+  static __device__ __forceinline__ int wo_holder(int tid) { return tid < WL - 1 ? tid : WL - 1; }
 };
-__device__ __forceinline__ float4 res_ld(const float4* res, int slot, int tid) { return res[slot * ROLE_NT + tid]; }
-__device__ __forceinline__ void res_st(float4* res, int slot, int tid, const float4& v) { res[slot * ROLE_NT + tid] = v; }
+__device__ __forceinline__ float4 res_ld(const float4* res, int base, int NH, int slot, int k) { return res[base + slot * NH + k]; }
+__device__ __forceinline__ void res_st(float4* res, int base, int NH, int slot, int k, const float4& v) { res[base + slot * NH + k] = v; }
 
 __device__ __forceinline__ float gelu_erf_f(float x) {
   return 0.5f * x * (1.0f + erff(x * 0.70710678118654752440f));
@@ -775,7 +782,7 @@
           for (int q = 0; q < RG::NRND; q++) {
             float4 wl[RK];
 #pragma unroll
-            for (int j = 0; j < RK; j++) wl[j] = res_ld(res, q * RK + j, tid);
+            for (int j = 0; j < RK; j++) wl[j] = res_ld(res, 0, RG::QL, q * RK + j, RG::q_holder(wave, lane));
             const int kb = RK * (2 + q);
 #pragma unroll
             for (int j = 0; j < RK; j++) {
@@ -902,7 +909,7 @@
   if constexpr (RG::NWO_A > 0) {
     if (res != nullptr) {
 #pragma unroll
-      for (int i = 0; i < RG::NWO_A; i++) wo[i] = res_ld(res, RG::WO_A + i, tid);
+      for (int i = 0; i < RG::NWO_A; i++) wo[i] = res_ld(res, RG::WO_A, RG::WL, i, RG::wo_holder(tid));
     }
   }
   float ov[4] = {0.f, 0.f, 0.f, 0.f};
@@ -953,7 +960,8 @@
 #pragma unroll
     for (int j = 0; j < RK; j++) w[j] = ld_w4(wq + (int64_t)(RK * (2 + q) + j) * a.ldqkv);
 #pragma unroll
-    for (int j = 0; j < RK; j++) res_st(res, q * RK + j, tid, w[j]);
+    for (int j = 0; j < RK; j++)
+      if (seg < 3) res_st(res, 0, RG::QL, q * RK + j, RG::q_holder(wave, lane), w[j]);
   }
   if constexpr (RG::NWO_A > 0) {
     const int cf = tid % CF, jg = tid / CF;
@@ -963,7 +971,8 @@
 #pragma unroll
     for (int i = 0; i < RG::NWO_A; i++) w[i] = ld_w4(wp + (int64_t)i * d);
 #pragma unroll
-    for (int i = 0; i < RG::NWO_A; i++) res_st(res, RG::WO_A + i, tid, w[i]);
+    for (int i = 0; i < RG::NWO_A; i++)
+      if (jg < G) res_st(res, RG::WO_A, RG::WL, i, tid, w[i]);
   }
 }
 
@@ -1202,7 +1211,7 @@
         for (int i = 0; i < SL; i++) {
           const int k0 = t * KT + rgp + 32 * i, key = p * PASS_C + k0;
           const float pk = key < C ? pbuf[key] : 0.f;
-          if (t < RG::NVT) { if (res_v) kv[t][i] = res_ld(res, t * SL + i, tid); }
+          if (t < RG::NVT) { if (res_v) kv[t][i] = res_ld(res, 0, ROLE_NT, t * SL + i, tid); }
           o.x += pk * kv[t][i].x; o.y += pk * kv[t][i].y; o.z += pk * kv[t][i].z; o.w += pk * kv[t][i].w;
           if (p + 1 < NP)
             kv[t][i] = gld4(Vh + (min(key + PASS_C, C - 1) * a.ldkv + c4));
@@ -1223,7 +1232,7 @@
   if constexpr (RG::NWO_X > 0) {
     if (res != nullptr) {
 #pragma unroll
-      for (int i = 0; i < RG::NWO_X; i++) wo[i] = res_ld(res, RG::WO_X + i, tid);
+      for (int i = 0; i < RG::NWO_X; i++) wo[i] = res_ld(res, RG::WO_X, RG::WL, i, RG::wo_holder(tid));
     }
   }
   float ov[4] = {0.f, 0.f, 0.f, 0.f};
@@ -1269,7 +1278,7 @@
 #pragma unroll
       for (int i = 0; i < SL; i++) v[i] = gld4(Vh + (min(t * KT + rg + 32 * i, C - 1) * a.ldkv + c4));
 #pragma unroll
-      for (int i = 0; i < SL; i++) res_st(res, t * SL + i, tid, v[i]);
+      for (int i = 0; i < SL; i++) res_st(res, 0, ROLE_NT, t * SL + i, tid, v[i]);
     }
   }
   if constexpr (RG::NWO_X > 0) {
@@ -1280,10 +1289,11 @@
 #pragma unroll
     for (int i = 0; i < RG::NWO_X; i++) w[i] = ld_w4(wp + (int64_t)i * d);
 #pragma unroll
-    for (int i = 0; i < RG::NWO_X; i++) res_st(res, RG::WO_X + i, tid, w[i]);
-  }
-}
-
-
-}
-}
+    for (int i = 0; i < RG::NWO_X; i++)
+      if (jg < G) res_st(res, RG::WO_X, RG::WL, i, tid, w[i]);
+  }
+}
+
+
+}
+}
diff --git a/whisper-burn_amd/csrc/decode_persist.hip b/whisper-burn_amd/csrc/decode_persist.hip
--- a/whisper-burn_amd/csrc/decode_persist.hip
+++ b/whisper-burn_amd/csrc/decode_persist.hip
@@ -404,7 +404,8 @@
   }
 }
 
-__global__ void ps_seed_kernel(const float* __restrict__ x, int n, void* gx, unsigned tag) {
+__global__ void ps_seed_kernel(const float* __restrict__ x, int n, void* gx, unsigned tag, int* ctl) {
+  if (blockIdx.x == 0 && threadIdx.x == 0) ctl[HX_STOP] = INT_MAX;
   const Buf16 b(gx);
   for (int i = blockIdx.x * blockDim.x + threadIdx.x; i < n; i += gridDim.x * blockDim.x) st_gran(b, (uint32_t)i, tag, x[i]);
 }
@@ -426,6 +427,21 @@
   WB_PS_INSTANCES(WB_PS_SLOTS)
 #undef WB_PS_SLOTS
   return 0;
+}
+
+bool dec_persist_resident_geometry(int d, int n_rows, int max_keys, int out[5]) {
+  if (!dec_persist_supported(d, n_rows, max_keys)) return false;
+  const int dpl = d / 64, mr = n_rows > 4 ? 8 : 4, np = max_keys > CROSS_FUSED_MAX_C ? 2 : 1;
+#define WB_PS_GEOM(DPL_, MR_, NP_)                                                            \
+  if (dpl == DPL_ && mr == MR_ && np == NP_) {                                                \
+    using RG = ResGeom<DPL_, NP_, PsArena<DPL_, MR_, NP_>::RS>;                               \
+    out[0] = PsArena<DPL_, MR_, NP_>::RS; out[1] = RG::NRND; out[2] = RG::NWO_A; out[3] = RG::NVT; out[4] = RG::NWO_X; \
+    if (PsArena<DPL_, MR_, NP_>::RS == 0) out[1] = out[2] = out[3] = out[4] = 0;              \
+    return true;                                                                              \
+  }
+  WB_PS_INSTANCES(WB_PS_GEOM)
+#undef WB_PS_GEOM
+  return false;
 }
 
 int ps_ctl_ints(int S, int n_layer) { return HX_HDR + (S + n_layer * S + 2 * n_layer + 8 + PS_NGO + 1) * HX_LINE; }
@@ -454,8 +470,8 @@
   return cus * 1;
 }
 
-void launch_ps_seed(hipStream_t st, const float* x, int n, void* gx, unsigned tag) {
-  hipLaunchKernelGGL(ps_seed_kernel, dim3((n + 255) / 256), dim3(256), 0, st, x, n, gx, tag);
+void launch_ps_seed(hipStream_t st, const float* x, int n, void* gx, unsigned tag, int* ctl) {
+  hipLaunchKernelGGL(ps_seed_kernel, dim3((n + 255) / 256), dim3(256), 0, st, x, n, gx, tag, ctl);
 }
 
 int launch_dec_persist(hipStream_t st, const PersistArgs& a, int grid) {
diff --git a/whisper-burn_amd/csrc/sample_chain.cpp b/whisper-burn_amd/csrc/sample_chain.cpp
--- a/whisper-burn_amd/csrc/sample_chain.cpp
+++ b/whisper-burn_amd/csrc/sample_chain.cpp
@@ -186,6 +186,14 @@
 
 int wb_session_graph_count(const wb_session* s) { return s ? (int)s->graphs.size() : 0; }
 int64_t wb_session_graph_captures(const wb_session* s) { return s ? s->n_captures : 0; }
+int wb_persist_resident_geometry(int32_t n_state, int32_t n_rows, int32_t max_keys, int32_t* out5) {
+  WB_REQUIRE(out5, WB_ERR_ARG, "wb_persist_resident_geometry: null argument");
+  int g[5] = {0, 0, 0, 0, 0};
+  WB_REQUIRE(dec_persist_resident_geometry(n_state, n_rows, max_keys, g), WB_ERR_SHAPE,
+             "wb_persist_resident_geometry: no persistent instance serves n_state %d with %d rows and %d keys", n_state, n_rows, max_keys);
+  for (int i = 0; i < 5; i++) out5[i] = g[i];
+  return WB_OK;
+}
 
 int wb_session_decode_sample(wb_session* s, const wb_decode_params* p, const wb_sample_params* sp, const int32_t* prompt,
                              int32_t prompt_len, const uint8_t* active, const int32_t* stream_ids, int32_t* out_tokens,
diff --git a/whisper-burn_amd/csrc/session.cpp b/whisper-burn_amd/csrc/session.cpp
--- a/whisper-burn_amd/csrc/session.cpp
+++ b/whisper-burn_amd/csrc/session.cpp
@@ -283,6 +283,7 @@
   if (host_block) (void)hipHostFree(host_block);
   if (guard_host) (void)hipHostFree(guard_host);
   if (pcm_stage) (void)hipHostFree(pcm_stage);
+  if (ps_pin) (void)hipHostFree(ps_pin);
   if (ev_seg) (void)hipEventDestroy(ev_seg);
   if (st2) (void)hipStreamDestroy(st2);
   if (st) (void)hipStreamDestroy(st);
diff --git a/whisper-burn_amd/csrc/session.h b/whisper-burn_amd/csrc/session.h
--- a/whisper-burn_amd/csrc/session.h
+++ b/whisper-burn_amd/csrc/session.h
@@ -37,6 +37,11 @@
   wb::DevMem ps_gx, ps_gpa, ps_gpc, ps_gp2, ps_gxn;
   unsigned ps_launches = 0;
   int ps_grid = -1;
+  std::vector<uint64_t> ps_setup_key;
+  std::vector<wb::PsRole> ps_roles_host;
+  int ps_setup_grid = 0, ps_setup_n_lg = 0, ps_setup_n_res = 0;
+  int* ps_pin = nullptr; size_t ps_pin_ints = 0;
+  bool ps_pin_busy = false;
   int n_tiles_v = 0, ct_v = 128;
   int ks_qkv = 1, ksl_qkv = 0, ks_o = 1, ksl_o = 0, ks_1 = 1, ksl_1 = 0, ks_2 = 1, ksl_2 = 0, ks_v = 1, ksl_v = 0;
   wb::DevMem bc_ctl, bc_topk;
diff --git a/whisper-burn_amd/csrc/switches.h b/whisper-burn_amd/csrc/switches.h
--- a/whisper-burn_amd/csrc/switches.h
+++ b/whisper-burn_amd/csrc/switches.h
@@ -42,6 +42,7 @@
   X(enc_trace, "WHISPER_HIP_ENC_TRACE", STR, nullptr, "directory for per-thread dumps of the encoder stages (developer)")            \
   X(ps_stamps, "WHISPER_HIP_PS_STAMPS", STR, nullptr, "file for the persistent kernel's role timeline (developer)")                  \
   X(persist_resident, "WHISPER_HIP_PERSIST_RESIDENT", STR, nullptr, "persistent kernel: step-invariant operands stay in LDS (on); 0: off; log: on + report") \
+  X(persist_setup, "WHISPER_HIP_PERSIST_SETUP", STR, nullptr, "persistent kernel: launch setup cached on the session (on); 0: built per call; log: on + report; 0log: both") \
   X(persist_inject_fail, "WHISPER_HIP_PERSIST_INJECT_FAIL", STR, nullptr, "test hook: \"launch\" = the cooperative launch is refused")
 
 #define WB_SW_DECL(fn, name, kind, dflt, what) bool fn();
diff --git a/whisper-burn_amd/whisper_burn_amd/_lib.py b/whisper-burn_amd/whisper_burn_amd/_lib.py
--- a/whisper-burn_amd/whisper_burn_amd/_lib.py
+++ b/whisper-burn_amd/whisper_burn_amd/_lib.py
@@ -147,6 +147,7 @@
     "wb_session_rewind": (C.c_int, [C.c_void_p]),
     "wb_session_graph_count": (C.c_int, [C.c_void_p]),
     "wb_session_graph_captures": (C.c_int64, [C.c_void_p]),
+    "wb_persist_resident_geometry": (C.c_int, [C.c_int32, C.c_int32, C.c_int32, c_int32_p]),
     "wb_session_decode_sample": (C.c_int, [C.c_void_p, C.POINTER(WbDecodeParams), C.POINTER(WbSampleParams), c_int32_p,
                                            C.c_int32, c_uint8_p, c_int32_p, c_int32_p, C.c_int32, c_int32_p, c_double_p,
                                            c_int32_p]),
```

Result: faster. 2287 x real-time, median of 6 (+2.1%).
